# zhudongmei/glusterfs

Measured on AMD Instinct MI355X. Metric: EC encode/decode user-data GB/s (4+2, 8+4) at 1/2/4/8 MI355X; % HBM roofline, higher is better.
Workload: dtype u8

## Files before the change

glusterfs_amd/csrc/ec_jit.hip:

```cpp
#include <hip/hip_runtime.h>

#include <dlfcn.h>
#include <fcntl.h>
#include <spawn.h>
#include <sys/wait.h>
#include <unistd.h>
#include <pthread.h>
#include <errno.h>
#include <stdarg.h>
#include <stdint.h>
#include <stdio.h>
#include <stdlib.h>
#include <string.h>

#include <atomic>
#include <chrono>
#include <condition_variable>
#include <deque>
#include <mutex>
#include <new>
#include <string>
#include <thread>
#include <vector>

#include "ec_device.h"
#include "ec_jit.h"

extern char **environ;

namespace {

using u32 = uint32_t;
constexpr int kMaxDev = 16;
constexpr size_t kEntries = 32;
constexpr uint64_t kMaxCreated = 256;


u32 gf_mul(u32 a, u32 b)
{
    u32 r = 0;
    while (b) {
        if (b & 1)
            r ^= a;
        a <<= 1;
        if (a & 0x100)
            a ^= 0x11D;
        b >>= 1;
    }
    return r;
}

u32 plane_mask(u32 c, int b)
{
    u32 m = 0;
    for (int j = 0; j < 8; ++j)
        m |= ((gf_mul(c, 1u << j) >> b) & 1u) << j;
    return m;
}

struct Gen {
    std::string s;
    u32 ops = 0;

    void line(const char *fmt, ...) __attribute__((format(printf, 2, 3)))
    {
        char buf[256];
        va_list ap, aq;
        va_start(ap, fmt);
        va_copy(aq, ap);
        const int n = vsnprintf(buf, sizeof buf, fmt, ap);
        va_end(ap);
        if (n >= (int)sizeof buf) {
            std::string big((size_t)n + 1, '\0');
            vsnprintf(&big[0], big.size(), fmt, aq);
            big.resize((size_t)n);
            s += big;
        } else if (n > 0) {
            s += buf;
        }
        va_end(aq);
        s += '\n';
    }
};

void emit_program(Gen &g, int w, u32 k, u32 T, const uint8_t *coef, u32 r0, u32 r1)
{
    const u32 ps = T * 64u;
    const u32 no = (r1 - r0) * 8;
    g.line("__device__ __forceinline__ void prog%d(u32 col, u32 *acc)", w);
    g.line("{");
    g.line("    asm volatile(\"\" : \"+v\"(col));");
    std::string decl = "    u32 x0, x1, x2, x3, x4, x5, x6, x7, n0, n1, n2, n3, n4, n5, n6, n7";
    for (u32 o = 0; o < no; ++o)
        decl += ", a" + std::to_string(o);
    g.line("%s;", decl.c_str());
    for (int b = 0; b < 8; ++b)
        g.line("    n%d = LDW(col + %uu);", b, (u32)b * ps);
    std::vector<bool> started(no, false);
    for (u32 p = 0; p < k; ++p) {
        g.line("    x0 = n0; x1 = n1; x2 = n2; x3 = n3; x4 = n4; x5 = n5; x6 = n6; x7 = n7;");
        if (p + 1 < k)
            for (int b = 0; b < 8; ++b)
                g.line("    n%d = LDW(col + %uu);", b, ((p + 1) * 8 + (u32)b) * ps);
        g.line("    __builtin_amdgcn_sched_barrier(0);");
        g.line("    {");
        std::vector<u32> masks(no);
        for (u32 o = 0; o < no; ++o)
            masks[o] = plane_mask(coef[(size_t)(r0 + o / 8) * k + p], (int)(o % 8));
        for (int h = 0; h < 2; ++h) {
            bool need[16] = {};
            for (u32 o = 0; o < no; ++o)
                need[(masks[o] >> (4 * h)) & 15] = true;
            bool have[16] = {};
            for (int j = 0; j < 4; ++j) {
                g.line("        const u32 t%d_%d = x%d;", h, 1 << j, 4 * h + j);
                have[1 << j] = true;
            }
            for (int pc = 2; pc <= 4; ++pc)
                for (int m = 1; m < 16; ++m) {
                    if (__builtin_popcount(m) != pc || !(need[m] || (pc == 2 && m == 3 && need[15])))
                        continue;
                    if (have[m])
                        continue;
                    int bits[4], nb = 0;
                    for (int j = 0; j < 4; ++j)
                        if (m >> j & 1)
                            bits[nb++] = 1 << j;
                    if (pc == 2)
                        g.line("        const u32 t%d_%d = t%d_%d ^ t%d_%d;", h, m, h, bits[0], h, bits[1]);
                    else if (pc == 3)
                        g.line("        const u32 t%d_%d = xr3(t%d_%d, t%d_%d, t%d_%d);", h, m, h, bits[0],
                               h, bits[1], h, bits[2]);
                    else
                        g.line("        const u32 t%d_15 = xr3(t%d_3, t%d_4, t%d_8);", h, h, h, h);
                    have[m] = true;
                    ++g.ops;
                }
        }
        for (u32 o = 0; o < no; ++o) {
            const u32 m0 = masks[o] & 15, m1 = masks[o] >> 4;
            char t0[16] = "", t1[16] = "";
            if (m0)
                snprintf(t0, sizeof t0, "t0_%u", m0);
            if (m1)
                snprintf(t1, sizeof t1, "t1_%u", m1);
            if (!m0 && !m1)
                continue;
            if (!started[o]) {
                if (m0 && m1) {
                    g.line("        a%u = %s ^ %s;", o, t0, t1);
                    ++g.ops;
                } else {
                    g.line("        a%u = %s;", o, m0 ? t0 : t1);
                }
                started[o] = true;
            } else if (m0 && m1) {
                g.line("        a%u = xr3(a%u, %s, %s);", o, o, t0, t1);
                ++g.ops;
            } else {
                g.line("        a%u ^= %s;", o, m0 ? t0 : t1);
                ++g.ops;
            }
        }
        g.line("    }");
        g.line("    __builtin_amdgcn_sched_barrier(0);");
    }
    for (u32 o = 0; o < no; ++o)
        g.line("    acc[%u] = %s;", o, started[o] ? ("a" + std::to_string(o)).c_str() : "0u");
    g.line("}");
}

const char *kPrologue = R"(
typedef unsigned int u32;
typedef unsigned long long u64;
typedef u32 v4u __attribute__((ext_vector_type(4)));
#define LDW(off) (*(const __attribute__((address_space(3))) u32 *)(off))
__device__ __forceinline__ u32 xr3(u32 a, u32 b, u32 c)
{
    return __builtin_amdgcn_bitop3_b32(a, b, c, 0x96);
}
struct JitArgs {
    const unsigned char *in[16];
    unsigned char *out[16];
    u64 in_stride, out_stride, nstripes;
    u64 contig;    /* out[r] = out[0] + r * 512 and out_stride = ROWS * 512 */
};
)";

const char *kBody = R"(
template <int LA>
__device__ __forceinline__ void body(const JitArgs &a)
{
    extern __shared__ __attribute__((aligned(16))) unsigned char lds[];
    constexpr u32 NW = T / 2u, PER = T / 2u, NT = NW * 64u;
    const u32 tid = threadIdx.x, lane = tid & 63u;
    const u32 wave = __builtin_amdgcn_readfirstlane(tid >> 6);
    const u64 t0 = (u64)blockIdx.x * T;
    /* the shipped tile kernels' staging (ec_kernels_impl.h stage_tile): input
     * p, plane b, stripe s at ((p * 8 + b) * T + s) * 64 */
    for (u32 ins = wave; ins < K * PER; ins += NW) {
        const u32 p = ins / PER, el = (ins % PER) * 64u + lane, seg = el >> 2;
        const u64 st = t0 + seg % T;
        if (st < a.nstripes) {
            const unsigned char *gp = a.in[p] + st * a.in_stride + (seg / T) * 64u + (el & 3u) * 16u;
            __builtin_amdgcn_global_load_lds((const __attribute__((address_space(1))) void *)gp,
                                             (__attribute__((address_space(3))) void *)(lds + ins * 1024u),
                                             16, 0, LA);
        }
    }
    /* every wave's LDS-DMA has landed before any wave reads the tile: the
     * hiprtc build of __syncthreads() waits only for lgkmcnt (the product
     * build adds vmcnt(0) itself), so the wait is explicit */
    __builtin_amdgcn_s_waitcnt(0x0070);          /* vmcnt(0) lgkmcnt(0) */
    __syncthreads();
    /* wave w: rows half (w & 1), stripes 4 * (w >> 1) .. + 3 */
    const u32 half = wave & 1u, s = (wave >> 1) * 4u + (lane >> 4), cc = lane & 15u;
    const u32 col = (u32)(unsigned long long)(lds + s * 64u + cc * 4u);
    u32 acc[NA];
    if (half == 0)
        prog0(col, acc);
    else
        prog1(col, acc);
    __syncthreads();
    /* stripe s, row r at (s * ROWS + r) * 512: a full decode's tile is then
     * its output as it lies in memory (ec_method_decode's stripe-major out) */
    unsigned char *ob = lds + s * (ROWS * 512u) + cc * 4u;
    const u32 rb = half == 0 ? 0u : R0;
    const u32 nr = half == 0 ? R0 : ROWS - R0;
#pragma unroll
    for (u32 o = 0; o < NA; ++o)
        if (o < nr * 8u)
            *(u32 *)(ob + (rb + o / 8u) * 512u + (o % 8u) * 64u) = acc[o];
    __syncthreads();
    const u64 left = a.nstripes - t0;
    const u32 ns = (u32)(left < T ? left : T);
    if (a.contig) {
        /* one run of ns * ROWS * 512 bytes */
        unsigned char *o = a.out[0] + t0 * a.out_stride;
        for (u32 i = tid * 16u; i < ns * ROWS * 512u; i += NT * 16u)
            __builtin_nontemporal_store(*(const v4u *)(lds + i), (v4u *)(o + i));
    } else {
        /* row by row: 512-byte runs, one per stripe (fragment-major outputs) */
        for (u32 r = 0; r < ROWS; ++r) {
            const u32 ss = tid >> 5, q = tid & 31u;
            if (ss < ns)
                __builtin_nontemporal_store(*(const v4u *)(lds + (ss * ROWS + r) * 512u + q * 16u),
                                            (v4u *)(a.out[r] + (t0 + ss) * a.out_stride + q * 16u));
        }
    }
}
extern "C" __global__ __launch_bounds__(T / 2 * 64) void ec_jit_combine(JitArgs a) { body<0>(a); }
extern "C" __global__ __launch_bounds__(T / 2 * 64) void ec_jit_combine_nt(JitArgs a) { body<2>(a); }
)";


struct Compiler {
    std::string path, why;
    bool ok = false;

    Compiler()
    {
        if (const char *e = getenv("EC_MI355X_JITC")) {
            path = e;
        } else {
            Dl_info di;
            if (dladdr((const void *)&ecd_jit_stats, &di) && di.dli_fname) {
                path = di.dli_fname;
                const size_t sl = path.rfind('/');
                path = (sl == std::string::npos ? std::string(".") : path.substr(0, sl)) +
                       "/ec_jitc";
            }
        }
        ok = !path.empty() && access(path.c_str(), X_OK) == 0;
        if (!ok)
            why = "compiler " + (path.empty() ? std::string("ec_jitc") : path) + " not found";
    }
};

Compiler &compiler()
{
    static Compiler *c = new Compiler;
    return *c;
}

bool read_file(const std::string &p, std::vector<char> &out)
{
    FILE *f = fopen(p.c_str(), "rb");
    if (!f)
        return false;
    char buf[1 << 16];
    size_t n;
    out.clear();
    while ((n = fread(buf, 1, sizeof buf, f)) > 0)
        out.insert(out.end(), buf, buf + n);
    fclose(f);
    return true;
}

int run_compiler(const std::string &src, std::vector<char> &code, std::string &log)
{
    Compiler &c = compiler();
    if (!c.ok) {
        log = c.why;
        return -ENOSYS;
    }
    const char *tmp = getenv("TMPDIR");
    std::string base = std::string(tmp && *tmp ? tmp : "/tmp") + "/ec_jit_XXXXXX";
    std::vector<char> name(base.begin(), base.end());
    name.push_back('\0');
    const int fd = mkstemp(name.data());
    if (fd < 0) {
        log = "mkstemp failed";
        return -EIO;
    }
    const std::string sp(name.data()), cp = sp + ".co", lp = sp + ".log";
    const bool wrote = write(fd, src.data(), src.size()) == (ssize_t)src.size();
    close(fd);
    int rc = -EIO;
    if (wrote) {
        posix_spawn_file_actions_t fa;
        posix_spawn_file_actions_init(&fa);
        posix_spawn_file_actions_addopen(&fa, 1, "/dev/null", O_WRONLY, 0);
        posix_spawn_file_actions_addopen(&fa, 2, lp.c_str(), O_WRONLY | O_CREAT | O_TRUNC, 0600);
        char *argv[] = {const_cast<char *>(c.path.c_str()), const_cast<char *>(sp.c_str()),
                        const_cast<char *>(cp.c_str()), nullptr};
        pid_t pid = -1;
        if (posix_spawn(&pid, c.path.c_str(), &fa, nullptr, argv, environ) == 0) {
            int st = 0;
            while (waitpid(pid, &st, 0) < 0 && errno == EINTR) {
            }
            if (WIFEXITED(st) && WEXITSTATUS(st) == 0 && read_file(cp, code) && !code.empty())
                rc = 0;
            else
                rc = WIFEXITED(st) && WEXITSTATUS(st) == 2 ? -ENOSYS : -EIO;
        } else {
            log = "posix_spawn of the compiler failed";
        }
        posix_spawn_file_actions_destroy(&fa);
        if (rc) {
            std::vector<char> l;
            if (read_file(lp, l))
                log += std::string(l.begin(), l.end());
        }
    }
    unlink(sp.c_str());
    unlink(cp.c_str());
    unlink(lp.c_str());
    return rc;
}


struct Key {
    u32 k = 0, rows = 0;
    uint8_t coef[ECJ_MAX * ECJ_MAX] = {};
    bool operator==(const Key &o) const
    {
        return k == o.k && rows == o.rows && !memcmp(coef, o.coef, (size_t)k * rows);
    }
};

enum { kQueued = 0, kReady = 1, kFailed = 2 };

struct Entry {
    Key key;
    std::atomic<int> state{kQueued};
    std::vector<char> code;
    hipModule_t mod[kMaxDev] = {};
    hipFunction_t fn[kMaxDev][2] = {};
    int load_failed[kMaxDev] = {};
    uint64_t last_use = 0;
};

struct Jit {
    std::mutex mu;
    std::condition_variable cv;
    std::vector<Entry *> entries;
    std::deque<Entry *> queue;
    bool worker = false;
    uint64_t tick = 0;
    uint64_t created = 0;
    std::atomic<uint64_t> compiled{0}, failed{0}, launches{0}, compile_us{0}, lookups{0};
    std::string last_log;
};

Jit &jit()
{
    static Jit *j = new Jit;
    return *j;
}

long env_long(const char *name, long dflt)
{
    const char *e = getenv(name);
    return e && *e ? strtol(e, nullptr, 10) : dflt;
}

bool jit_on()
{
    static const bool v = env_long("EC_MI355X_JIT", 1) != 0;
    return v;
}

bool jit_sync()
{
    static const bool v = env_long("EC_MI355X_JIT_SYNC", 0) != 0;
    return v;
}

constexpr u32 kJitTile = 4;
u32 jit_tile()
{
    return kJitTile;
}

uint64_t jit_min_stripes()
{
    static const uint64_t v = (uint64_t)env_long("EC_MI355X_JIT_MIN_STRIPES", 1024);
    return v;
}

std::string source_of(const Key &key, u32 *ops)
{
    Gen g;
    const u32 r0 = (key.rows + 1) / 2;
    g.s += kPrologue;
    g.line("#define K %uu", key.k);
    g.line("#define ROWS %uu", key.rows);
    g.line("#define R0 %uu", r0);
    g.line("#define NA %uu", r0 * 8);
    g.line("#define T %uu", jit_tile());

    emit_program(g, 0, key.k, jit_tile(), key.coef, 0, r0);
    emit_program(g, 1, key.k, jit_tile(), key.coef, r0, key.rows);
    g.s += kBody;
    if (ops)
        *ops = g.ops;
    return g.s;
}

void compile_entry(Entry *e)
{
    Jit &j = jit();
    const auto t0 = std::chrono::steady_clock::now();
    u32 ops = 0;
    const std::string src = source_of(e->key, &ops);
    std::string log;
    const int st = run_compiler(src, e->code, log) == 0 ? kReady : kFailed;
    j.compile_us += (uint64_t)std::chrono::duration_cast<std::chrono::microseconds>(
                        std::chrono::steady_clock::now() - t0).count();
    (st == kReady ? j.compiled : j.failed)++;
    if (st != kReady) {
        std::lock_guard<std::mutex> g(j.mu);
        j.last_log = log.substr(0, 2000);
    }
    e->state.store(st, std::memory_order_release);
}

std::thread *g_worker;
bool g_stop;

void worker_main()
{
    Jit &j = jit();
    for (;;) {
        Entry *e;
        {
            std::unique_lock<std::mutex> g(j.mu);
            j.cv.wait(g, [&] { return g_stop || !j.queue.empty(); });
            if (g_stop)
                return;
            e = j.queue.front();
            j.queue.pop_front();
        }
        compile_entry(e);
    }
}

void fork_prepare()
{
    jit().mu.lock();
}

void fork_parent()
{
    jit().mu.unlock();
}

void fork_child()
{
    Jit &j = jit();
    new (&j.mu) std::mutex();
    new (&j.cv) std::condition_variable();
    j.queue.clear();
    j.worker = false;
    g_worker = nullptr;
}

Entry *lookup(const Key &key)
{
    Jit &j = jit();
    Entry *fresh = nullptr;
    {
        std::lock_guard<std::mutex> g(j.mu);
        for (Entry *e : j.entries)
            if (e->key == key) {
                e->last_use = ++j.tick;
                return e;
            }
        if (j.entries.size() >= kEntries) {
            size_t lru = j.entries.size();
            for (size_t i = 0; i < j.entries.size(); ++i)
                if (j.entries[i]->state.load() != kQueued &&
                    (lru == j.entries.size() || j.entries[i]->last_use < j.entries[lru]->last_use))
                    lru = i;
            if (lru == j.entries.size())
                return nullptr;
            j.entries.erase(j.entries.begin() + (long)lru);
        }
        if (j.created >= kMaxCreated)
            return nullptr;
        ++j.created;
        fresh = new Entry;
        fresh->key = key;
        fresh->last_use = ++j.tick;
        j.entries.push_back(fresh);
        if (!jit_sync()) {
            j.queue.push_back(fresh);
            if (!j.worker) {
                static std::once_flag once;
                std::call_once(once, [] { pthread_atfork(fork_prepare, fork_parent, fork_child); });
                g_worker = new std::thread(worker_main);
                j.worker = true;
            }
            j.cv.notify_one();
        }
    }
    if (jit_sync())
        compile_entry(fresh);
    return fresh;
}

hipFunction_t function_of(Entry *e, bool nt)
{
    int dev = 0;
    if (hipGetDevice(&dev) != hipSuccess || dev < 0 || dev >= kMaxDev) {
        (void)hipGetLastError();
        return nullptr;
    }
    Jit &j = jit();
    std::lock_guard<std::mutex> g(j.mu);
    if (e->load_failed[dev])
        return nullptr;
    if (!e->mod[dev]) {
        hipModule_t m = nullptr;
        hipFunction_t f0 = nullptr, f1 = nullptr;
        if (hipModuleLoadData(&m, e->code.data()) != hipSuccess ||
            hipModuleGetFunction(&f0, m, "ec_jit_combine") != hipSuccess ||
            hipModuleGetFunction(&f1, m, "ec_jit_combine_nt") != hipSuccess) {
            (void)hipGetLastError();
            e->load_failed[dev] = 1;
            return nullptr;
        }
        e->mod[dev] = m;
        e->fn[dev][0] = f0;
        e->fn[dev][1] = f1;
    }
    return e->fn[dev][nt ? 1 : 0];
}

struct JitArgs {
    const uint8_t *in[16];
    uint8_t *out[16];
    uint64_t in_stride, out_stride, nstripes;
    uint64_t contig;
};

}

extern "C" int ecj_lds_pad_kb = 0;

extern "C" int ecj_eligible(const ecd_combine_desc_t *d)
{
    if (!jit_on() || d->npatterns != 1 || d->group_pattern || d->k < 12 || d->k > ECJ_MAX ||
        d->rows < 12 || d->rows > ECJ_MAX || d->nstripes < jit_min_stripes() ||
        d->nstripes / 4 + 1 > 0x7fffffffull)
        return 0;
    if (d->out_stride % 16)
        return 0;
    for (uint32_t r = 0; r < d->rows; ++r)
        if (!d->out_base[r] || ((uintptr_t)d->out_base[r] & 15))
            return 0;
    return 1;
}

extern "C" int ecj_launch(hipStream_t s, const ecd_combine_desc_t *d, int nt)
{
    if (!ecj_eligible(d) || !compiler().ok)
        return -EAGAIN;
    const uint8_t *pat = d->pat_ext ? d->pat_ext : d->pat;
    Key key;
    key.k = d->k;
    key.rows = d->rows;
    memcpy(key.coef, pat + d->k, (size_t)d->rows * d->k);
    jit().lookups++;
    Entry *e = lookup(key);
    if (!e || e->state.load(std::memory_order_acquire) != kReady)
        return -EAGAIN;
    hipFunction_t f = function_of(e, nt != 0);
    if (!f)
        return -EAGAIN;
    JitArgs a;
    memset(&a, 0, sizeof a);
    for (uint32_t p = 0; p < d->k; ++p) {
        a.in[p] = static_cast<const uint8_t *>(d->in_base[pat[p]]);
        if (!a.in[p])
            return -EAGAIN;
    }
    for (uint32_t r = 0; r < d->rows; ++r)
        a.out[r] = static_cast<uint8_t *>(d->out_base[r]);
    a.in_stride = d->in_stride;
    a.out_stride = d->out_stride;
    a.nstripes = d->nstripes;
    a.contig = d->out_stride == (uint64_t)d->rows * 512;
    for (uint32_t r = 1; r < d->rows && a.contig; ++r)
        a.contig = a.out[r] == a.out[0] + (size_t)r * 512;
    const u32 T = jit_tile();
    const size_t lds = (size_t)(d->k > d->rows ? d->k : d->rows) * T * 512 +
                       (size_t)ecj_lds_pad_kb * 1024;
    if (lds > (64u << 10))
        return -EAGAIN;
    void *params[] = {&a};
    const hipError_t rc = hipModuleLaunchKernel(f, (u32)((d->nstripes + T - 1) / T), 1, 1, T / 2 * 64,
                                                1, 1, (u32)lds, s, params, nullptr);
    if (rc != hipSuccess) {
        (void)hipGetLastError();
        return -EAGAIN;
    }
    jit().launches++;
    return 0;
}

extern "C" void ecd_jit_stats(ecd_jit_stats_t *st)
{
    Jit &j = jit();
    st->compiled = j.compiled.load();
    st->failed = j.failed.load();
    st->launches = j.launches.load();
    st->compile_us = j.compile_us.load();
    st->lookups = j.lookups.load();
    std::lock_guard<std::mutex> g(j.mu);
    st->entries = j.entries.size();
}

extern "C" int ecd_jit_prepare(uint32_t k, uint32_t rows, const uint8_t *coef)
{
    if (k < 1 || k > ECJ_MAX || rows < 2 || rows > ECJ_MAX || !coef)
        return -EINVAL;
    if (!jit_on())
        return -EPERM;
    if (!compiler().ok)
        return -ENOSYS;
    Key key;
    key.k = k;
    key.rows = rows;
    memcpy(key.coef, coef, (size_t)k * rows);
    return lookup(key) ? 0 : -ENOSPC;
}

extern "C" int ecd_jit_source(uint32_t k, uint32_t rows, const uint8_t *coef, char *buf, size_t len)
{
    if (k < 1 || k > ECJ_MAX || rows < 2 || rows > ECJ_MAX || !coef)
        return -EINVAL;
    Key key;
    key.k = k;
    key.rows = rows;
    memcpy(key.coef, coef, (size_t)k * rows);
    const std::string src = source_of(key, nullptr);
    if (buf && len) {
        const size_t n = src.size() < len - 1 ? src.size() : len - 1;
        memcpy(buf, src.data(), n);
        buf[n] = '\0';
    }
    return (int)(src.size() + 1);
}

extern "C" int ecd_jit_compile_check(uint32_t k, uint32_t rows, const uint8_t *coef, uint32_t *ops,
                                 char *log, size_t log_len)
{
    if (k < 1 || k > ECJ_MAX || rows < 2 || rows > ECJ_MAX || !coef)
        return -EINVAL;
    if (!compiler().ok) {
        if (log && log_len)
            snprintf(log, log_len, "%s", compiler().why.c_str());
        return -ENOSYS;
    }
    Entry e;
    e.key.k = k;
    e.key.rows = rows;
    memcpy(e.key.coef, coef, (size_t)k * rows);
    const std::string src = source_of(e.key, ops);
    compile_entry(&e);
    if (const char *d = getenv("EC_MI355X_JIT_DUMP")) {
        if (FILE *f = fopen((std::string(d) + ".hip").c_str(), "w")) {
            fwrite(src.data(), 1, src.size(), f);
            fclose(f);
        }
        if (!e.code.empty())
            if (FILE *f = fopen((std::string(d) + ".co").c_str(), "wb")) {
                fwrite(e.code.data(), 1, e.code.size(), f);
                fclose(f);
            }
    }
    if (e.state.load() != kReady && log && log_len) {
        std::lock_guard<std::mutex> g(jit().mu);
        snprintf(log, log_len, "%s", jit().last_log.c_str());
    }
    return e.state.load() == kReady ? (int)e.code.size() : -EIO;
}
```

Measured before the change: 3323.

## Extend JIT GF(2^8) combine kernel to narrow k<=8 codes with row groups and searched XOR programs

Result: slower. 3193 (-3.9%).

```diff
diff --git a/glusterfs_amd/csrc/ec_gf8_prog_tab.h b/glusterfs_amd/csrc/ec_gf8_prog_tab.h
--- /dev/null
+++ b/glusterfs_amd/csrc/ec_gf8_prog_tab.h
@@ -0,0 +1,281 @@
+#ifndef EC_MI355X_GF8_PROG_TAB_H
+#define EC_MI355X_GF8_PROG_TAB_H
+
+static const unsigned short ecgf_prog_off[256] = {
+    0, 0, 17, 37, 66, 90, 121, 152, 189, 215, 249, 281, 320, 351, 391, 430,
+    469, 499, 528, 564, 602, 635, 672, 712, 752, 786, 823, 860, 898, 936, 976, 1016,
+    1057, 1091, 1123, 1153, 1181, 1218, 1253, 1293, 1325, 1362, 1398, 1434, 1469, 1507, 1548, 1587,
+    1626, 1660, 1697, 1733, 1771, 1809, 1848, 1884, 1923, 1960, 1996, 2034, 2071, 2114, 2152, 2192,
+    2231, 2267, 2302, 2339, 2368, 2405, 2436, 2463, 2487, 2524, 2562, 2598, 2636, 2676, 2712, 2744,
+    2778, 2815, 2849, 2886, 2920, 2957, 2997, 3028, 3066, 3105, 3143, 3182, 3221, 3257, 3298, 3335,
+    3374, 3409, 3447, 3486, 3527, 3563, 3600, 3641, 3680, 3719, 3759, 3799, 3837, 3870, 3906, 3945,
+    3983, 4019, 4056, 4091, 4128, 4165, 4201, 4238, 4276, 4317, 4358, 4394, 4431, 4471, 4511, 4550,
+    4588, 4626, 4667, 4700, 4739, 4776, 4816, 4845, 4883, 4920, 4960, 4993, 5031, 5060, 5096, 5116,
+    5145, 5183, 5222, 5258, 5298, 5335, 5375, 5413, 5450, 5490, 5529, 5565, 5601, 5634, 5667, 5699,
+    5732, 5772, 5811, 5848, 5887, 5927, 5964, 5997, 6032, 6069, 6103, 6146, 6185, 6214, 6241, 6276,
+    6309, 6350, 6388, 6426, 6463, 6500, 6541, 6578, 6613, 6649, 6687, 6727, 6765, 6803, 6842, 6880,
+    6922, 6956, 6989, 7026, 7064, 7105, 7142, 7184, 7222, 7257, 7288, 7327, 7365, 7405, 7444, 7483,
+    7525, 7564, 7603, 7644, 7682, 7722, 7757, 7794, 7832, 7861, 7896, 7931, 7970, 8009, 8044, 8083,
+    8121, 8158, 8195, 8231, 8271, 8306, 8343, 8383, 8421, 8460, 8500, 8533, 8569, 8606, 8644, 8680,
+    8718, 8756, 8796, 8837, 8873, 8909, 8943, 8983, 9016, 9056, 9097, 9137, 9170, 9208, 9246, 9285,
+};
+
+static const signed char ecgf_prog_tab[] = {
+     0, 1, 0, 1, 1, 1, 2, 1, 3, 1, 4, 1, 5, 1, 6, 1, 7,
+     0, 1, 7, 1, 0, 2, 7, 1, 2, 7, 2, 2, 7, 3, 1, 4, 1, 5, 1, 6,
+     1, 2, 7, -1, 2, 7, 0, 2, 1, 0, 2, 8, 1, 2, 8, 3, 3, 7, 4, 3, 2, 5, 4, 2, 6, 5, 2, 7, 6,
+     1, 6, 7, -1, 1, 6, 1, 7, 2, 6, 0, 2, 8, 1, 2, 8, 2, 2, 7, 3, 1, 4, 1, 5,
+     0, 2, 6, 0, 2, 7, 1, 3, 6, 2, 0, 4, 7, 6, 3, 1, 4, 7, 6, 4, 2, 3, 7, 5, 3, 2, 6, 4, 2, 7, 5,
+     1, 2, 6, -1, 2, 7, 6, 2, 7, 0, 4, 7, 6, 1, 0, 2, 8, 1, 2, 8, 3, 3, 7, 4, 3, 2, 5, 4, 2, 6, 5,
+     4, 6, 7, -1, 0, 1, 8, 2, 3, 6, 4, 5, 7, 2, 8, 0, 2, 9, 6, 2, 9, 2, 2, 10, 1, 2, 10, 4, 2, 11, 3, 2, 11, 8, 2, 8, 5,
+     0, 1, 5, 1, 6, 2, 7, 5, 3, 6, 5, 0, 4, 7, 6, 5, 1, 3, 7, 6, 2, 2, 7, 3, 1, 4,
+     2, 2, 5, 7, 6, 7, -1, 2, 5, 0, 2, 6, 1, 1, 8, 4, 6, 5, 3, 0, 4, 9, 5, 4, 1, 2, 8, 6, 2, 9, 3, 2, 7, 4,
+     1, 2, 6, 7, 2, 7, 5, 2, 6, 0, 2, 5, 1, 3, 8, 5, 0, 4, 6, 5, 3, 1, 2, 8, 4, 3, 7, 5, 3, 2, 6, 4,
+     3, 5, 6, 7, 4, 8, -1, 0, 6, -1, 2, 10, 8, 2, 10, 1, 3, 5, 2, 1, 4, 8, 3, 2, 0, 4, 9, 7, 3, 1, 2, 9, 2, 2, 8, 3, 2, 9, 5,
+     1, 0, 5, 7, 2, 6, 5, 2, 7, 6, 2, 8, 6, 2, 8, 1, 3, 5, 2, 1, 3, 6, 3, 2, 3, 7, 4, 3, 2, 5, 4,
+     4, 5, 7, -1, 0, 6, 8, 1, 2, 5, 1, 3, 6, 2, 9, 7, 3, 7, 6, 1, 2, 9, 2, 2, 11, 9, 2, 10, 4, 2, 11, 10, 4, 11, 7, 4, 1, 2, 8, 4,
+     4, 0, 1, 5, 5, 6, -1, 1, 7, 9, 2, 3, 6, 2, 10, 1, 2, 10, 8, 2, 8, 6, 2, 8, 2, 2, 11, 10, 2, 11, 4, 4, 7, 5, 4, 3, 2, 9, 4,
+     4, 5, 6, 7, 0, 1, 5, 3, 4, 8, 2, 9, -1, 2, 8, 0, 2, 9, 8, 2, 11, 6, 2, 11, 3, 4, 10, 6, 2, 1, 3, 10, 7, 2, 1, 10, 2, 10, 3,
+     2, 4, 5, 6, 6, 7, -1, 1, 4, 1, 5, 2, 6, 4, 2, 9, 8, 2, 8, 0, 3, 9, 5, 1, 2, 9, 2, 2, 7, 3,
+     0, 2, 4, 0, 2, 5, 1, 3, 6, 4, 2, 4, 7, 5, 4, 3, 3, 6, 5, 0, 3, 7, 6, 1, 2, 7, 2, 1, 3,
+     4, 5, 6, 7, 1, 4, 8, 1, 3, 9, 4, 5, -1, 2, 7, 4, 2, 5, 0, 2, 9, 5, 2, 11, 2, 2, 10, 0, 1, 9, 2, 8, 2, 2, 11, 10,
+     4, 0, 5, -1, 4, 7, -1, 1, 6, 9, 2, 4, 5, 2, 9, 0, 2, 8, 1, 2, 10, 2, 2, 11, 3, 4, 8, 7, 6, 3, 1, 10, 2, 11, 9, 2, 6, 3,
+     2, 1, 5, 6, 2, 4, 7, 2, 6, 4, 2, 7, 5, 2, 4, 0, 2, 8, 4, 3, 9, 5, 0, 2, 8, 3, 2, 9, 6, 3, 7, 5, 3,
+     4, 0, 4, -1, 0, 2, 7, 1, 5, -1, 3, 6, 10, 2, 8, 6, 2, 10, 7, 2, 8, 2, 2, 11, 4, 2, 9, 5, 2, 11, 5, 2, 9, 8, 2, 5, 3,
+     4, 4, 5, -1, 5, 6, 7, 0, 4, 7, 2, 4, 9, 2, 9, 8, 2, 10, 8, 2, 10, 1, 2, 11, 1, 4, 8, 3, 2, 0, 4, 8, 6, 3, 1, 1, 11, 2, 9, 3,
+     4, 2, 4, 7, 1, 8, -1, 3, 5, 6, 0, 2, 6, 2, 11, 8, 4, 7, 5, 1, 0, 2, 9, 0, 2, 10, 9, 2, 11, 10, 4, 6, 4, 3, 1, 2, 8, 5, 1, 10,
+     2, 4, 6, 7, 3, 6, -1, 2, 5, 4, 2, 6, 5, 2, 8, 5, 2, 8, 0, 4, 7, 4, 1, 0, 3, 5, 2, 1, 2, 9, 2, 2, 9, 8,
+     4, 0, 4, -1, 6, 7, 8, 0, 5, 9, 1, 4, 7, 2, 8, 5, 2, 11, 10, 2, 10, 2, 2, 9, 3, 2, 11, 8, 2, 2, 1, 2, 3, 2, 2, 4, 3,
+     4, 0, 1, 4, 0, 5, 6, 2, 4, 5, 3, 4, 6, 3, 10, 7, 2, 1, 9, 2, 9, 8, 2, 10, 9, 2, 8, 3, 2, 10, 1, 2, 11, 10, 2, 11, 7,
+     3, 2, 4, -1, 1, 5, 6, 3, 6, 8, 4, 7, 5, 4, 0, 2, 9, 0, 2, 9, 8, 2, 10, 0, 3, 3, 1, 0, 2, 8, 1, 3, 5, 3, 2, 2, 10, 2,
+     4, 4, 5, 7, 4, 6, -1, 0, 1, 9, 2, 3, 4, 2, 9, 5, 2, 9, 8, 2, 8, 0, 2, 10, 6, 2, 10, 2, 3, 11, 8, 1, 2, 11, 6, 2, 8, 3,
+     4, 0, 4, 5, 3, 4, -1, 1, 3, 8, 2, 7, 8, 2, 8, 6, 4, 7, 6, 5, 1, 1, 11, 2, 10, 5, 4, 6, 2, 1, 0, 2, 11, 10, 2, 9, 2, 2, 9, 5,
+     4, 2, 4, -1, 5, 6, 7, 3, 8, 9, 0, 1, 5, 2, 9, 4, 2, 9, 0, 2, 11, 4, 4, 8, 7, 1, 0, 2, 11, 10, 3, 10, 6, 1, 2, 10, 7, 2, 10, 2,
+     5, 0, 1, 7, 2, 3, 8, 3, 4, 5, 9, 10, -1, 2, 6, 11, 2, 12, 1, 2, 12, 4, 2, 11, 7, 2, 9, 4, 2, 9, 6, 3, 9, 4, 0, 2, 10, 2, 2, 10, 6,
+     1, 3, 5, -1, 2, 7, 3, 1, 4, 2, 8, 7, 4, 7, 6, 4, 3, 2, 8, 4, 4, 6, 5, 4, 0, 4, 7, 6, 5, 1, 3, 7, 6, 2,
+     1, 4, 6, -1, 3, 7, 3, 0, 2, 4, 1, 4, 7, 5, 3, 2, 2, 8, 7, 2, 5, 3, 2, 8, 0, 3, 7, 5, 1, 2, 6, 2,
+     0, 1, 3, 2, 4, 0, 3, 5, 3, 1, 4, 6, 4, 3, 2, 3, 7, 5, 4, 3, 6, 5, 0, 3, 7, 6, 1, 2, 7, 2,
+     0, 2, 3, 0, 3, 4, 1, 0, 4, 5, 3, 2, 1, 3, 6, 4, 2, 2, 7, 5, 2, 6, 0, 2, 7, 1, 1, 2,
+     4, 5, 6, 7, 1, 4, -1, 3, 4, 8, 1, 9, 10, 2, 11, 5, 2, 7, 4, 2, 11, 0, 2, 9, 3, 2, 10, 2, 2, 10, 0, 2, 9, 8, 2, 8, 2,
+     4, 3, 6, 7, 1, 4, 7, 2, 5, -1, 0, 8, -1, 1, 11, 1, 9, 2, 11, 10, 2, 4, 1, 2, 10, 8, 2, 11, 4, 2, 9, 5, 2, 10, 6,
+     4, 0, 3, 5, 4, 7, -1, 1, 6, -1, 2, 4, 5, 2, 6, 3, 2, 9, 0, 2, 10, 8, 4, 9, 3, 2, 1, 2, 11, 6, 3, 8, 7, 6, 2, 10, 9, 2, 11, 9,
+     2, 0, 3, 6, 1, 4, 7, 1, 8, 2, 9, 0, 4, 8, 5, 2, 1, 2, 9, 2, 3, 6, 5, 2, 2, 8, 7, 1, 9, 2, 5, 2,
+     3, 3, 7, -1, 4, 5, 8, 1, 5, 6, 2, 9, 4, 2, 6, 4, 1, 3, 2, 9, 0, 2, 10, 9, 4, 9, 3, 2, 0, 2, 10, 3, 4, 7, 6, 4, 2,
+     2, 0, 4, 7, 4, 6, -1, 4, 7, 5, 3, 0, 2, 9, 1, 2, 3, 2, 2, 8, 5, 4, 7, 6, 3, 1, 2, 8, 2, 3, 5, 3, 1, 2, 9, 2,
+     3, 0, 2, 5, 1, 3, -1, 4, 6, -1, 2, 5, 3, 2, 10, 0, 2, 9, 7, 3, 8, 4, 3, 2, 10, 1, 2, 8, 7, 2, 9, 6, 3, 7, 4, 2,
+     2, 0, 3, -1, 2, 3, 7, 2, 8, 5, 4, 6, 4, 1, 0, 2, 9, 1, 4, 5, 4, 2, 0, 2, 6, 1, 2, 9, 8, 2, 3, 1, 2, 4, 2,
+     4, 3, 5, 6, 2, 3, 4, 0, 5, -1, 1, 4, 8, 2, 8, 7, 3, 7, 6, 4, 2, 10, 8, 2, 11, 0, 2, 9, 1, 2, 10, 9, 1, 11, 3, 9, 8, 7,
+     4, 0, 2, 3, 0, 1, -1, 1, 3, 5, 4, 5, 6, 4, 10, 9, 7, 6, 4, 7, 6, 4, 1, 2, 8, 6, 2, 11, 9, 2, 9, 8, 2, 8, 4, 2, 10, 4, 2, 11, 2,
+     4, 1, 3, 6, 2, 4, 7, 0, 2, 6, 1, 5, 8, 1, 11, 2, 10, 9, 3, 8, 7, 0, 4, 11, 9, 1, 0, 2, 9, 1, 2, 11, 10, 2, 8, 4, 2, 9, 5,
+     4, 1, 7, -1, 0, 6, 8, 2, 3, -1, 2, 4, 5, 4, 6, 5, 3, 0, 2, 9, 4, 2, 10, 9, 2, 11, 9, 2, 8, 2, 2, 10, 0, 3, 4, 3, 1, 1, 11,
+     2, 3, 6, -1, 4, 7, 8, 2, 9, 6, 2, 5, 4, 2, 9, 5, 2, 8, 5, 2, 8, 0, 4, 7, 4, 1, 0, 3, 5, 2, 1, 2, 8, 2,
+     3, 0, 4, 7, 3, 6, 7, 1, 5, -1, 2, 8, 3, 2, 10, 4, 4, 9, 5, 4, 2, 2, 6, 5, 2, 9, 8, 2, 10, 8, 3, 10, 6, 2, 2, 9, 2,
+     3, 0, 7, -1, 4, 5, -1, 3, 6, 9, 2, 4, 3, 2, 9, 0, 2, 10, 1, 4, 10, 7, 4, 2, 2, 8, 6, 2, 8, 1, 2, 2, 1, 2, 3, 2,
+     4, 1, 2, 6, 1, 5, 7, 0, 4, 7, 3, 7, -1, 2, 11, 10, 2, 10, 9, 4, 8, 5, 4, 3, 2, 9, 8, 2, 10, 6, 2, 9, 0, 1, 8, 2, 11, 2,
+     5, 4, 5, 7, 1, 3, 4, 3, 5, 6, 0, 3, 8, 2, 4, 5, 2, 10, 8, 1, 8, 1, 11, 2, 9, 8, 2, 12, 11, 2, 9, 0, 2, 12, 1, 2, 10, 2,
+     5, 3, 4, 7, 0, 8, -1, 1, 5, 7, 2, 5, -1, 4, 6, 11, 2, 9, 6, 2, 10, 4, 2, 11, 9, 1, 10, 2, 9, 2, 2, 10, 9, 2, 12, 1, 2, 12, 8,
+     4, 2, 3, 5, 3, 4, -1, 1, 5, 9, 0, 4, 5, 2, 9, 6, 2, 11, 7, 2, 10, 0, 2, 8, 1, 2, 2, 0, 2, 11, 10, 2, 10, 8, 1, 8,
+     3, 0, 3, 4, 1, 5, 8, 2, 8, -1, 2, 8, 6, 3, 9, 7, 3, 2, 9, 2, 2, 10, 9, 2, 10, 3, 2, 9, 4, 4, 6, 4, 2, 1, 4, 7, 5, 3, 2,
+     3, 3, 5, 7, 4, 6, -1, 1, 8, -1, 2, 8, 4, 2, 9, 5, 2, 9, 3, 2, 3, 0, 2, 10, 0, 4, 9, 2, 1, 0, 2, 10, 2, 3, 9, 3, 2,
+     4, 1, 4, 5, 2, 3, 6, 0, 3, 8, 4, 7, 9, 3, 10, 7, 1, 2, 8, 6, 2, 9, 4, 1, 0, 2, 10, 7, 2, 10, 9, 2, 11, 8, 1, 11,
+     2, 3, 4, -1, 2, 3, 7, 2, 8, 5, 4, 6, 5, 4, 0, 4, 8, 7, 6, 1, 2, 9, 0, 3, 5, 1, 0, 4, 6, 2, 1, 0, 2, 9, 1, 2, 8, 2,
+     4, 0, 4, 5, 1, 6, -1, 2, 4, 9, 3, 7, 10, 2, 8, 3, 2, 9, 8, 1, 11, 3, 7, 2, 0, 2, 8, 1, 2, 10, 8, 2, 11, 4, 2, 11, 9,
+     6, 3, 4, -1, 6, 7, 8, 2, 5, 6, 0, 1, 9, 1, 3, 10, 3, 9, -1, 2, 9, 5, 2, 13, 5, 2, 8, 0, 2, 11, 4, 2, 12, 0, 2, 11, 2, 2, 13, 12, 2, 10, 8,
+     4, 4, 5, 6, 0, 2, 3, 7, 8, 9, 1, 10, -1, 2, 10, 2, 2, 11, 9, 2, 9, 4, 4, 7, 6, 1, 0, 2, 11, 7, 1, 11, 2, 11, 0, 2, 10, 0,
+     5, 0, 1, 3, 2, 6, 8, 4, 7, -1, 0, 6, 10, 3, 4, 5, 2, 12, 6, 2, 11, 5, 2, 10, 8, 1, 9, 3, 12, 10, 9, 2, 9, 7, 2, 11, 9, 2, 12, 2,
+     4, 0, 1, 6, 4, 7, 8, 2, 3, 9, 5, 10, -1, 4, 11, 7, 2, 1, 2, 9, 5, 2, 10, 6, 2, 8, 2, 2, 11, 3, 2, 11, 4, 2, 10, 0, 2, 11, 8,
+     2, 2, 6, 7, 3, 4, -1, 1, 8, 2, 7, 3, 2, 8, 4, 4, 6, 5, 3, 2, 2, 9, 2, 2, 9, 5, 4, 6, 5, 4, 0, 4, 8, 5, 2, 1,
+     3, 5, 6, -1, 0, 4, -1, 0, 6, 7, 2, 10, 2, 3, 7, 3, 1, 2, 10, 9, 2, 8, 2, 2, 3, 2, 2, 4, 3, 2, 9, 5, 2, 8, 1,
+     4, 0, 6, -1, 3, 6, 7, 1, 2, 4, 1, 7, -1, 2, 6, 2, 2, 9, 8, 2, 10, 6, 2, 9, 5, 2, 11, 10, 2, 5, 3, 2, 8, 4, 2, 11, 5,
+     0, 3, 6, 2, 0, 4, 7, 3, 1, 0, 3, 6, 4, 1, 3, 7, 6, 5, 2, 7, 2, 1, 3, 2, 4, 0, 2, 5, 1,
+     3, 1, 7, -1, 0, 4, 7, 0, 5, -1, 2, 7, 2, 1, 3, 2, 9, 2, 4, 8, 5, 3, 2, 4, 9, 6, 3, 0, 2, 10, 9, 2, 10, 6, 2, 8, 6,
+     1, 0, 7, -1, 2, 8, 2, 2, 3, 1, 2, 8, 4, 4, 7, 5, 2, 1, 3, 7, 6, 3, 2, 7, 4, 2, 5, 0, 2, 6, 1,
+     0, 1, 2, 2, 3, 0, 4, 4, 2, 1, 0, 3, 5, 3, 1, 2, 6, 4, 2, 7, 5, 2, 6, 0, 2, 7, 1,
+     1, 0, 1, -1, 2, 2, 0, 2, 8, 3, 2, 8, 4, 2, 5, 1, 1, 6, 1, 7, 1, 0, 1, 1,
+     4, 4, 5, 6, 2, 7, 8, 0, 2, 3, 1, 9, -1, 2, 9, 4, 3, 7, 6, 3, 2, 8, 2, 1, 10, 2, 11, 3, 2, 9, 3, 2, 10, 9, 2, 11, 2,
+     3, 3, 6, 7, 4, 5, 6, 0, 8, -1, 4, 10, 5, 3, 2, 2, 8, 1, 1, 9, 2, 2, 0, 4, 8, 5, 2, 1, 3, 8, 4, 2, 2, 10, 9, 2, 9, 1,
+     4, 2, 5, 6, 0, 3, 7, 1, 4, 7, 7, 8, -1, 1, 8, 2, 9, 6, 2, 10, 8, 1, 9, 2, 11, 10, 2, 11, 3, 3, 9, 6, 4, 2, 10, 5,
+     4, 0, 3, 7, 0, 2, 6, 1, 5, 6, 4, 10, -1, 2, 9, 5, 3, 8, 6, 1, 2, 11, 7, 2, 7, 0, 2, 10, 2, 2, 9, 8, 2, 8, 4, 2, 11, 6,
+     3, 0, 3, 6, 2, 4, 5, 5, 7, -1, 2, 10, 2, 2, 8, 0, 2, 9, 0, 4, 8, 7, 2, 1, 4, 9, 3, 2, 1, 2, 9, 6, 2, 10, 8, 4, 7, 6, 4, 1,
+     2, 1, 6, -1, 0, 2, 7, 2, 9, 5, 2, 8, 3, 3, 5, 4, 0, 2, 9, 8, 3, 5, 3, 1, 3, 6, 4, 2, 4, 7, 5, 3, 0, 2, 8, 4,
+     2, 0, 3, 6, 1, 4, 7, 2, 5, 2, 1, 8, 4, 9, 5, 2, 0, 2, 8, 1, 2, 9, 5, 3, 6, 5, 2, 2, 8, 7, 1, 9,
+     3, 0, 1, 6, 0, 5, -1, 1, 7, 9, 2, 9, 2, 2, 8, 3, 2, 10, 4, 1, 8, 2, 10, 0, 2, 6, 2, 3, 7, 3, 0, 2, 4, 1,
+     4, 3, 5, 6, 5, 7, -1, 4, 8, 9, 0, 2, 8, 3, 10, 3, 2, 2, 9, 3, 2, 7, 2, 2, 10, 2, 1, 11, 2, 10, 1, 2, 11, 10, 2, 8, 1,
+     4, 2, 4, 6, 3, 5, 7, 0, 7, 8, 1, 6, 9, 1, 10, 2, 9, 1, 1, 7, 2, 10, 0, 2, 10, 9, 2, 11, 4, 2, 10, 5, 1, 11,
+     3, 0, 5, 7, 4, 6, -1, 2, 4, 8, 2, 9, 2, 2, 8, 3, 2, 2, 1, 2, 9, 3, 2, 10, 9, 4, 7, 6, 3, 1, 2, 10, 5, 3, 5, 3, 1,
+     4, 0, 2, 4, 1, 3, 5, 6, 7, 8, 7, 9, -1, 2, 8, 6, 2, 11, 0, 1, 1, 2, 6, 4, 2, 10, 5, 2, 11, 6, 1, 10, 1, 11,
+     4, 0, 5, 7, 1, 3, 4, 4, 6, -1, 2, 6, 7, 2, 11, 10, 2, 5, 3, 2, 11, 0, 2, 9, 2, 2, 8, 3, 2, 10, 1, 2, 8, 2, 2, 10, 9,
+     4, 0, 7, -1, 2, 4, -1, 1, 3, 6, 3, 4, 5, 2, 9, 8, 3, 5, 3, 1, 2, 8, 6, 2, 9, 1, 2, 11, 8, 2, 11, 10, 4, 8, 6, 5, 2, 2, 10, 7,
+     0, 2, 4, 2, 3, 5, 3, 0, 4, 6, 2, 1, 0, 4, 7, 4, 3, 1, 2, 5, 0, 2, 6, 1, 3, 7, 2, 0, 2, 3, 1,
+     3, 0, 4, -1, 1, 6, -1, 1, 7, -1, 2, 8, 2, 4, 5, 3, 1, 0, 2, 9, 0, 2, 10, 4, 2, 8, 5, 2, 9, 5, 4, 7, 6, 2, 0, 2, 10, 3,
+     4, 2, 3, 4, 3, 5, 6, 0, 5, 8, 1, 4, -1, 3, 9, 8, 7, 2, 9, 7, 2, 5, 2, 2, 10, 7, 4, 11, 8, 7, 0, 2, 8, 1, 1, 10, 2, 11, 9,
+     5, 0, 2, 4, 1, 3, 7, 5, 6, 9, 7, 8, 10, 6, 11, -1, 2, 11, 9, 1, 10, 1, 5, 2, 12, 9, 2, 9, 8, 2, 12, 0, 2, 11, 1, 2, 10, 4,
+     5, 0, 3, 5, 2, 4, 5, 1, 2, 3, 0, 10, -1, 7, 8, -1, 2, 9, 6, 2, 12, 6, 2, 12, 11, 2, 8, 4, 2, 11, 3, 1, 10, 2, 9, 8, 2, 10, 9,
+     4, 0, 2, 4, 1, 3, 5, 5, 8, -1, 7, 9, -1, 2, 10, 6, 3, 11, 6, 0, 2, 11, 3, 2, 10, 2, 2, 8, 1, 2, 9, 2, 3, 8, 6, 3, 2, 11, 4,
+     3, 0, 2, 5, 1, 3, 6, 2, 4, 7, 2, 10, 5, 3, 9, 5, 1, 2, 8, 6, 3, 9, 8, 4, 2, 9, 0, 2, 10, 1, 2, 8, 3, 2, 9, 4,
+     4, 1, 4, 5, 3, 5, 6, 0, 9, -1, 7, 8, -1, 4, 11, 2, 1, 0, 2, 9, 1, 2, 10, 3, 4, 8, 6, 2, 0, 2, 10, 8, 2, 11, 2, 2, 10, 2, 2, 11, 9,
+     3, 0, 5, 6, 1, 7, 8, 3, 4, -1, 3, 5, 4, 2, 2, 8, 3, 2, 9, 2, 2, 10, 9, 2, 9, 5, 3, 7, 2, 1, 3, 3, 2, 0, 2, 10, 1,
+     5, 1, 5, 7, 0, 6, 8, 0, 2, 3, 3, 4, 5, 3, 9, -1, 2, 11, 10, 2, 12, 7, 1, 9, 2, 9, 4, 2, 12, 11, 2, 8, 2, 2, 10, 6, 2, 11, 8,
+     2, 3, 6, -1, 2, 4, 5, 2, 8, 2, 3, 7, 4, 3, 2, 9, 8, 2, 9, 7, 2, 5, 2, 2, 8, 0, 4, 7, 4, 1, 0, 3, 5, 2, 1,
+     4, 0, 3, 6, 3, 4, 5, 1, 5, 7, 2, 9, -1, 2, 8, 2, 2, 10, 9, 2, 9, 6, 2, 11, 7, 2, 11, 3, 2, 8, 5, 3, 10, 9, 8, 2, 10, 2,
+     4, 2, 3, 7, 0, 3, 4, 1, 2, 5, 8, 10, -1, 2, 8, 6, 2, 9, 7, 4, 11, 6, 4, 2, 2, 5, 4, 2, 8, 5, 2, 9, 6, 2, 11, 9, 2, 10, 6,
+     5, 4, 5, 7, 3, 8, -1, 1, 6, 8, 0, 1, 9, 7, 10, 11, 2, 12, 2, 2, 11, 5, 2, 10, 3, 2, 9, 7, 2, 9, 2, 2, 12, 8, 2, 10, 0, 3, 10, 4, 2,
+     3, 0, 7, -1, 5, 6, -1, 2, 4, 9, 2, 3, 2, 2, 4, 3, 4, 10, 6, 3, 0, 2, 10, 1, 2, 9, 7, 2, 8, 6, 2, 8, 1, 2, 2, 1,
+     3, 0, 6, 7, 0, 4, 5, 0, 2, 3, 1, 10, 3, 4, 3, 1, 2, 9, 3, 4, 10, 9, 6, 1, 2, 9, 8, 2, 8, 5, 2, 8, 1, 3, 7, 2, 1,
+     5, 1, 5, 7, 4, 8, -1, 0, 3, 9, 1, 6, -1, 3, 5, 11, 3, 7, 3, 2, 2, 10, 8, 2, 10, 2, 2, 9, 6, 2, 12, 1, 2, 12, 10, 2, 8, 0, 2, 11, 2,
+     5, 1, 6, 7, 3, 4, 5, 0, 3, 7, 1, 4, 10, 6, 9, -1, 2, 10, 2, 2, 11, 7, 2, 11, 5, 2, 9, 8, 1, 12, 2, 12, 10, 2, 12, 11, 2, 8, 2,
+     4, 4, 6, 7, 1, 2, 4, 0, 2, 3, 0, 8, -1, 4, 10, 6, 5, 0, 2, 8, 3, 2, 11, 10, 2, 11, 2, 2, 9, 8, 2, 10, 7, 2, 10, 9, 2, 9, 5,
+     5, 1, 4, -1, 3, 6, 7, 0, 2, 9, 2, 7, 8, 5, 10, -1, 2, 12, 7, 2, 9, 8, 2, 9, 4, 2, 10, 4, 2, 11, 6, 2, 12, 6, 2, 11, 10, 2, 11, 5,
+     4, 4, 6, -1, 2, 3, 6, 1, 2, 8, 0, 7, 8, 3, 9, 7, 5, 2, 11, 3, 2, 10, 3, 2, 8, 0, 2, 9, 1, 2, 11, 9, 4, 10, 9, 5, 0, 2, 10, 5,
+     4, 1, 4, 6, 0, 3, 8, 2, 5, 7, 0, 3, 10, 2, 11, 6, 2, 9, 7, 2, 9, 0, 2, 9, 1, 3, 9, 2, 0, 2, 11, 4, 2, 9, 5, 2, 10, 8,
+     3, 1, 2, 4, 2, 3, -1, 0, 4, 9, 2, 9, 5, 3, 6, 4, 3, 2, 10, 7, 2, 8, 0, 1, 1, 2, 2, 0, 2, 10, 8, 1, 8,
+     3, 0, 1, 3, 0, 2, 5, 1, 4, 7, 2, 9, 3, 4, 8, 6, 4, 0, 2, 10, 8, 3, 8, 4, 2, 2, 4, 1, 1, 9, 2, 8, 6, 2, 10, 2,
+     3, 0, 1, 3, 1, 4, 6, 2, 4, -1, 4, 7, 5, 3, 2, 2, 9, 8, 2, 10, 8, 4, 7, 4, 1, 0, 3, 8, 7, 0, 2, 10, 0, 2, 8, 5, 2, 9, 2,
+     5, 1, 3, 4, 0, 8, -1, 0, 2, 5, 3, 7, 10, 5, 6, 9, 1, 11, 2, 12, 5, 1, 9, 2, 9, 7, 2, 8, 7, 2, 10, 4, 2, 12, 4, 2, 12, 11,
+     4, 2, 4, 6, 3, 5, 7, 0, 1, -1, 2, 9, -1, 2, 8, 3, 2, 9, 4, 2, 11, 7, 1, 2, 2, 8, 0, 2, 10, 9, 2, 10, 8, 2, 11, 1,
+     3, 0, 2, 4, 1, 3, 5, 6, 8, -1, 2, 10, 3, 3, 9, 7, 4, 2, 9, 1, 2, 3, 2, 2, 10, 4, 4, 7, 3, 1, 0, 2, 8, 1, 2, 9, 2,
+     4, 2, 3, 7, 1, 5, 8, 0, 2, 9, 4, 6, 8, 1, 11, 3, 10, 4, 1, 1, 9, 1, 7, 2, 11, 0, 2, 10, 4, 2, 11, 10, 2, 9, 6,
+     4, 0, 3, 7, 0, 1, 5, 2, 6, 8, 1, 4, 8, 2, 10, 4, 2, 11, 5, 2, 9, 8, 2, 8, 0, 1, 10, 1, 11, 3, 9, 4, 2, 3, 10, 9, 7,
+     3, 0, 2, 6, 1, 2, 7, 3, 4, -1, 2, 10, 2, 2, 10, 5, 3, 8, 5, 3, 2, 9, 6, 3, 7, 4, 0, 3, 5, 1, 0, 2, 8, 1, 2, 9, 3,
+     1, 1, 2, -1, 4, 4, 3, 2, 0, 4, 5, 4, 3, 1, 4, 6, 5, 3, 0, 4, 8, 7, 6, 3, 2, 7, 0, 2, 1, 0, 2, 8, 0, 2, 8, 3,
+     4, 0, 1, 5, 2, 3, 7, 0, 3, 4, 6, 8, -1, 2, 9, 4, 2, 10, 5, 2, 11, 9, 2, 6, 1, 1, 10, 2, 8, 4, 2, 11, 2, 3, 9, 6, 1,
+     4, 0, 4, -1, 1, 3, 6, 1, 2, 5, 2, 3, 8, 2, 11, 7, 2, 11, 10, 4, 9, 7, 5, 0, 1, 9, 2, 3, 0, 2, 8, 1, 2, 10, 0, 2, 9, 2,
+     5, 2, 3, 7, 4, 5, 8, 6, 9, -1, 0, 1, 3, 2, 5, 6, 2, 10, 7, 2, 10, 2, 1, 8, 2, 12, 0, 2, 11, 9, 2, 12, 11, 4, 10, 5, 1, 0, 2, 9, 1,
+     5, 0, 2, 3, 1, 8, -1, 5, 6, 8, 3, 7, 9, 4, 11, -1, 2, 10, 4, 2, 12, 10, 2, 7, 3, 1, 10, 2, 11, 5, 2, 9, 6, 2, 12, 3, 4, 9, 5, 4, 0,
+     4, 1, 2, 3, 4, 5, 8, 6, 7, 9, 0, 8, 10, 2, 10, 1, 2, 11, 3, 1, 8, 2, 11, 4, 2, 9, 0, 3, 9, 6, 0, 2, 10, 0, 1, 10,
+     4, 0, 3, 5, 1, 2, 8, 4, 6, 9, 7, 10, -1, 2, 11, 1, 2, 11, 2, 2, 3, 1, 3, 8, 7, 6, 1, 9, 2, 10, 5, 2, 11, 6, 2, 10, 0,
+     4, 1, 2, 7, 0, 6, 8, 3, 4, 5, 5, 8, -1, 2, 10, 2, 2, 10, 6, 3, 9, 3, 1, 2, 11, 0, 4, 11, 9, 4, 1, 2, 9, 5, 2, 9, 3, 2, 11, 10,
+     5, 1, 2, 3, 0, 7, 8, 0, 1, 5, 0, 3, 6, 4, 10, -1, 2, 12, 8, 2, 12, 11, 2, 11, 7, 2, 9, 5, 2, 10, 6, 3, 11, 9, 0, 1, 9, 2, 8, 4,
+     4, 0, 5, -1, 3, 6, 8, 1, 2, 9, 4, 7, 10, 4, 11, 6, 1, 0, 2, 9, 4, 2, 10, 5, 2, 8, 1, 2, 11, 2, 2, 11, 3, 2, 11, 4, 2, 11, 8,
+     4, 0, 3, 5, 1, 6, 8, 2, 7, 8, 0, 4, 9, 2, 10, 4, 2, 11, 0, 2, 9, 5, 2, 8, 1, 2, 9, 7, 2, 11, 10, 2, 10, 1, 3, 11, 5, 2,
+     4, 3, 4, -1, 1, 2, 5, 2, 6, 7, 1, 3, 6, 2, 10, 9, 1, 10, 2, 11, 5, 2, 9, 4, 2, 11, 10, 2, 8, 2, 2, 8, 5, 4, 6, 5, 4, 0,
+     4, 1, 2, -1, 3, 4, 5, 6, 7, -1, 0, 5, 10, 2, 11, 1, 2, 10, 8, 4, 8, 6, 5, 3, 2, 9, 8, 4, 8, 7, 4, 3, 2, 9, 2, 2, 9, 6, 2, 11, 4,
+     0, 3, 6, 5, 1, 4, 7, 6, 2, 0, 4, 7, 6, 5, 3, 4, 7, 5, 4, 1, 2, 2, 1, 2, 3, 2, 2, 4, 3, 3, 5, 4, 0,
+     4, 2, 7, -1, 3, 5, 8, 0, 1, 6, 1, 2, 4, 2, 10, 5, 2, 10, 8, 2, 9, 6, 2, 11, 9, 1, 11, 2, 9, 7, 3, 6, 4, 3, 4, 7, 5, 4, 0,
+     4, 5, 7, -1, 2, 4, 8, 0, 1, 3, 0, 6, -1, 2, 8, 1, 2, 6, 2, 2, 10, 5, 2, 9, 6, 2, 11, 10, 2, 9, 5, 2, 5, 3, 2, 11, 4,
+     4, 2, 4, 7, 3, 5, 6, 0, 2, 6, 1, 10, -1, 4, 7, 5, 1, 0, 2, 11, 0, 2, 11, 9, 2, 9, 8, 4, 6, 4, 3, 1, 2, 8, 5, 1, 9, 2, 10, 8,
+     0, 2, 5, 1, 3, 6, 2, 0, 4, 7, 5, 3, 0, 3, 6, 5, 4, 3, 7, 6, 1, 2, 7, 2, 1, 3, 2, 4, 0,
+     4, 0, 5, -1, 2, 7, 8, 0, 1, 6, 0, 4, 7, 2, 8, 1, 2, 10, 2, 2, 9, 3, 4, 6, 5, 4, 3, 2, 11, 10, 2, 9, 0, 2, 6, 3, 1, 11,
+     4, 0, 6, -1, 1, 6, 7, 3, 5, 6, 4, 5, 7, 1, 9, 2, 7, 2, 2, 9, 3, 4, 8, 4, 2, 1, 2, 10, 2, 2, 11, 10, 1, 11, 2, 8, 5,
+     4, 5, 6, 7, 2, 7, -1, 0, 1, 6, 3, 4, 8, 2, 10, 7, 2, 9, 1, 4, 10, 9, 3, 0, 4, 10, 4, 3, 2, 2, 11, 9, 1, 11, 2, 11, 3, 2, 8, 0,
+     1, 0, 7, -1, 2, 6, 1, 2, 8, 2, 2, 6, 3, 4, 8, 6, 4, 1, 4, 7, 6, 5, 2, 3, 7, 6, 3, 2, 7, 4, 2, 5, 0,
+     3, 2, 6, -1, 0, 1, 2, 4, 7, 8, 2, 9, 8, 2, 9, 7, 2, 8, 3, 3, 10, 9, 3, 2, 10, 5, 4, 7, 6, 5, 3, 2, 10, 2, 3, 7, 5, 0,
+     0, 2, 7, 1, 1, 2, 4, 7, 3, 1, 0, 4, 7, 4, 2, 0, 3, 7, 5, 3, 2, 6, 4, 2, 7, 5, 2, 6, 0,
+     3, 0, 7, -1, 2, 3, 8, 5, 6, -1, 2, 8, 1, 2, 2, 1, 2, 9, 1, 2, 9, 4, 4, 7, 5, 4, 3, 2, 10, 4, 2, 10, 7, 2, 8, 6,
+     0, 1, 1, 2, 2, 0, 2, 3, 0, 2, 4, 0, 1, 5, 1, 6, 1, 7, 1, 0,
+     1, 0, 2, -1, 2, 1, 0, 2, 8, 1, 2, 8, 3, 3, 4, 3, 0, 2, 5, 4, 2, 6, 5, 2, 7, 6, 2, 7, 0,
+     4, 3, 4, 5, 6, 7, 8, 1, 2, -1, 2, 3, 9, 2, 11, 10, 2, 11, 4, 2, 8, 1, 2, 10, 7, 3, 10, 9, 0, 2, 10, 9, 2, 9, 2, 2, 9, 0,
+     4, 1, 2, 7, 5, 8, -1, 3, 4, 9, 0, 6, 10, 3, 11, 3, 2, 2, 9, 6, 2, 10, 7, 2, 8, 3, 2, 11, 4, 3, 11, 5, 0, 2, 10, 1, 2, 11, 8,
+     4, 2, 5, 6, 3, 4, 7, 1, 4, 8, 5, 9, -1, 2, 10, 2, 3, 8, 7, 0, 1, 11, 1, 1, 2, 10, 0, 2, 10, 9, 2, 11, 8, 2, 11, 0,
+     5, 1, 6, -1, 0, 5, 8, 2, 3, 7, 2, 7, -1, 3, 4, 5, 2, 9, 4, 2, 11, 9, 2, 12, 11, 2, 3, 1, 2, 9, 2, 2, 10, 8, 2, 10, 4, 2, 12, 0,
+     4, 1, 4, 5, 2, 6, -1, 0, 3, 8, 3, 7, 9, 2, 8, 7, 2, 9, 5, 2, 10, 6, 1, 9, 1, 10, 2, 9, 8, 2, 11, 5, 4, 11, 4, 2, 0,
+     4, 0, 1, 5, 1, 2, 6, 1, 3, 9, 4, 8, -1, 2, 11, 7, 2, 9, 5, 2, 11, 10, 1, 10, 2, 8, 3, 2, 9, 4, 4, 7, 5, 3, 2, 4, 10, 4, 2, 0,
+     3, 0, 4, 7, 1, 5, -1, 2, 5, 6, 2, 9, 4, 2, 10, 0, 4, 10, 8, 3, 2, 2, 7, 6, 2, 9, 8, 2, 10, 1, 4, 7, 6, 3, 2, 2, 8, 3,
+     3, 0, 1, 5, 2, 6, -1, 3, 7, 9, 2, 8, 4, 2, 9, 8, 4, 10, 5, 4, 0, 2, 10, 2, 2, 8, 7, 2, 9, 1, 2, 10, 6, 3, 4, 3, 0,
+     4, 1, 3, 4, 2, 5, 6, 0, 2, 3, 7, 9, -1, 4, 7, 6, 4, 1, 2, 11, 6, 2, 8, 7, 3, 11, 1, 0, 2, 10, 4, 2, 8, 5, 2, 9, 4, 2, 11, 10,
+     4, 1, 4, -1, 1, 2, 5, 0, 3, 6, 3, 7, 8, 2, 11, 10, 2, 9, 7, 2, 11, 2, 3, 10, 9, 7, 3, 3, 2, 0, 2, 8, 3, 2, 9, 8, 2, 10, 5,
+     2, 0, 2, 7, 4, 6, -1, 2, 9, 1, 2, 8, 5, 2, 4, 3, 4, 6, 5, 1, 0, 2, 8, 4, 3, 5, 3, 1, 2, 9, 2, 4, 7, 5, 3, 0,
+     2, 0, 5, -1, 2, 7, 8, 4, 6, 4, 1, 0, 2, 9, 1, 3, 4, 3, 2, 4, 8, 6, 3, 1, 2, 9, 5, 2, 3, 1, 2, 4, 2, 2, 8, 3,
+     3, 0, 3, 6, 1, 4, 7, 2, 5, -1, 1, 9, 1, 10, 2, 9, 8, 2, 10, 0, 3, 9, 8, 1, 2, 9, 5, 2, 10, 6, 2, 8, 7,
+     2, 0, 3, 6, 1, 4, 7, 2, 9, 0, 3, 5, 2, 1, 3, 9, 8, 2, 4, 5, 3, 2, 0, 2, 8, 7, 1, 9, 2, 5, 2, 1, 8,
+     2, 0, 4, 6, 0, 5, -1, 2, 4, 1, 2, 9, 2, 2, 8, 3, 2, 9, 7, 1, 8, 3, 7, 5, 1, 2, 6, 2, 3, 7, 3, 0,
+     1, 0, 4, -1, 2, 8, 1, 4, 5, 2, 1, 0, 4, 8, 6, 3, 2, 4, 7, 5, 3, 0, 2, 6, 0, 2, 7, 1, 1, 2, 2, 3, 0,
+     5, 2, 5, 6, 4, 6, 7, 1, 9, -1, 0, 8, -1, 1, 3, 8, 2, 12, 2, 2, 9, 2, 2, 10, 4, 2, 12, 7, 2, 10, 8, 2, 11, 3, 2, 10, 3, 2, 11, 9,
+     5, 1, 2, 7, 6, 8, -1, 0, 2, 3, 3, 4, 7, 5, 7, 10, 2, 12, 9, 2, 9, 4, 1, 9, 2, 9, 5, 2, 8, 5, 2, 10, 6, 2, 11, 1, 2, 12, 11,
+     4, 1, 3, 5, 4, 6, 7, 0, 2, 9, 4, 8, -1, 2, 11, 9, 1, 10, 1, 6, 2, 8, 6, 2, 11, 2, 4, 10, 8, 7, 1, 2, 9, 8, 2, 10, 5,
+     4, 0, 2, 6, 1, 3, 5, 4, 8, -1, 7, 8, 9, 2, 11, 2, 3, 10, 7, 1, 2, 8, 0, 3, 6, 5, 1, 2, 9, 2, 2, 10, 3, 2, 11, 10, 2, 10, 5,
+     3, 0, 7, -1, 2, 4, -1, 3, 5, -1, 2, 10, 1, 2, 9, 6, 2, 8, 1, 2, 10, 2, 4, 6, 5, 4, 1, 4, 8, 6, 5, 2, 4, 7, 6, 3, 1, 2, 9, 8,
+     3, 0, 2, 7, 1, 6, -1, 2, 4, -1, 4, 5, 3, 1, 0, 2, 10, 9, 2, 8, 1, 2, 5, 2, 2, 9, 5, 2, 8, 6, 3, 7, 3, 1, 2, 10, 0,
+     4, 3, 5, 7, 0, 2, 4, 1, 6, 8, 6, 7, 9, 2, 8, 1, 2, 9, 6, 1, 0, 1, 8, 2, 10, 4, 2, 11, 5, 1, 10, 1, 11,
+     4, 0, 2, 4, 1, 3, 5, 6, 8, -1, 7, 9, -1, 2, 11, 0, 2, 10, 1, 2, 2, 0, 2, 7, 5, 2, 11, 6, 2, 10, 7, 1, 11, 1, 10,
+     3, 1, 6, -1, 0, 2, 7, 2, 4, -1, 2, 8, 3, 2, 10, 7, 2, 8, 5, 3, 9, 3, 1, 2, 10, 6, 4, 7, 5, 3, 0, 2, 8, 4, 2, 9, 5,
+     3, 1, 2, 7, 0, 1, 6, 0, 2, 5, 2, 9, 3, 2, 8, 4, 2, 10, 9, 2, 8, 0, 2, 6, 2, 3, 7, 3, 0, 2, 4, 1, 1, 10,
+     6, 6, 7, -1, 0, 4, 7, 1, 3, -1, 0, 2, 5, 1, 5, 6, 9, 10, 12, 2, 10, 8, 2, 9, 2, 2, 8, 5, 2, 10, 0, 2, 13, 11, 2, 13, 6, 2, 12, 4, 2, 11, 8,
+     4, 0, 4, 7, 1, 8, -1, 2, 6, 7, 0, 5, 7, 4, 9, 6, 4, 3, 2, 9, 2, 2, 10, 5, 2, 1, 0, 2, 10, 3, 2, 8, 3, 2, 11, 9, 2, 11, 10,
+     0, 2, 3, 1, 2, 4, 2, 3, 5, 1, 0, 4, 6, 3, 2, 0, 2, 7, 4, 2, 5, 0, 2, 6, 1, 3, 7, 2, 0,
+     0, 3, 3, 1, 0, 3, 4, 2, 1, 4, 5, 2, 1, 0, 3, 6, 2, 0, 1, 7, 1, 0, 1, 1, 2, 2, 0,
+     3, 0, 4, -1, 0, 6, 7, 5, 6, -1, 3, 7, 3, 1, 2, 8, 2, 2, 10, 9, 2, 9, 3, 2, 4, 3, 2, 8, 5, 2, 10, 1, 2, 9, 2,
+     1, 0, 6, -1, 4, 7, 3, 1, 0, 4, 4, 2, 1, 0, 4, 7, 5, 2, 0, 2, 8, 7, 1, 3, 2, 4, 0, 2, 5, 1, 2, 8, 2,
+     5, 1, 2, -1, 3, 4, 8, 0, 7, 8, 2, 5, 6, 4, 7, -1, 2, 11, 9, 2, 12, 11, 2, 12, 1, 2, 9, 6, 2, 10, 6, 2, 10, 3, 1, 9, 4, 9, 5, 1, 0,
+     4, 1, 4, 6, 0, 3, 5, 2, 7, 8, 1, 9, 10, 2, 9, 8, 2, 10, 5, 2, 10, 6, 2, 8, 2, 2, 10, 0, 2, 11, 8, 3, 8, 3, 2, 2, 11, 6,
+     5, 1, 3, 4, 0, 2, 6, 6, 7, 8, 4, 5, 9, 5, 8, -1, 2, 10, 5, 2, 11, 7, 1, 4, 1, 10, 2, 12, 11, 2, 10, 9, 2, 12, 2, 2, 11, 3,
+     4, 1, 4, 6, 0, 2, 8, 3, 5, 9, 7, 10, -1, 2, 11, 2, 2, 11, 3, 2, 4, 2, 2, 8, 7, 2, 9, 3, 2, 11, 6, 2, 10, 0, 2, 11, 1,
+     3, 1, 2, -1, 2, 3, 4, 2, 4, 6, 3, 9, 8, 5, 2, 10, 5, 4, 10, 8, 7, 0, 2, 9, 7, 2, 1, 0, 2, 8, 0, 2, 8, 3, 2, 9, 0,
+     4, 2, 4, -1, 0, 1, 2, 0, 3, 7, 6, 7, 9, 4, 9, 8, 5, 3, 4, 8, 6, 5, 1, 2, 11, 4, 2, 8, 7, 2, 9, 8, 2, 9, 5, 2, 11, 10, 2, 10, 8,
+     3, 0, 2, 4, 6, 8, -1, 1, 3, 5, 3, 10, 7, 4, 2, 9, 5, 2, 9, 2, 2, 4, 3, 4, 7, 3, 1, 0, 2, 8, 1, 2, 10, 2, 2, 9, 3,
+     4, 0, 1, 4, 1, 2, 6, 3, 7, 8, 2, 5, 8, 2, 10, 5, 2, 11, 6, 2, 9, 8, 1, 4, 1, 10, 1, 11, 3, 9, 5, 3, 2, 10, 9,
+     3, 0, 2, 5, 1, 3, 4, 2, 4, 7, 2, 9, 6, 2, 10, 5, 3, 5, 4, 1, 2, 9, 8, 1, 8, 4, 6, 3, 1, 0, 2, 10, 1, 2, 8, 3,
+     5, 2, 4, 5, 1, 8, -1, 0, 2, 3, 6, 9, 10, 5, 7, 10, 2, 11, 5, 2, 9, 7, 1, 9, 2, 9, 0, 2, 8, 0, 2, 11, 4, 2, 12, 11, 1, 12,
+     5, 2, 5, -1, 4, 7, 8, 0, 3, 8, 1, 9, 10, 6, 11, -1, 2, 12, 0, 2, 9, 0, 2, 9, 2, 2, 11, 5, 2, 10, 7, 2, 12, 7, 2, 9, 1, 2, 10, 6,
+     4, 4, 5, 7, 0, 1, 8, 3, 6, 9, 0, 2, 3, 2, 10, 5, 2, 9, 2, 2, 8, 2, 1, 9, 2, 11, 8, 2, 10, 7, 2, 11, 10, 4, 10, 4, 2, 1,
+     4, 0, 6, 7, 4, 5, -1, 1, 2, 7, 2, 8, 9, 3, 4, 3, 1, 2, 9, 2, 2, 11, 10, 2, 11, 3, 2, 8, 5, 2, 8, 1, 1, 10, 3, 3, 2, 0,
+     4, 0, 1, 4, 1, 6, 7, 2, 5, 8, 5, 9, -1, 2, 8, 3, 2, 10, 0, 2, 10, 6, 2, 10, 9, 2, 11, 8, 2, 11, 0, 2, 9, 2, 4, 7, 3, 2, 0,
+     4, 0, 4, 5, 6, 8, -1, 0, 3, 6, 1, 5, 7, 3, 11, 10, 9, 2, 8, 2, 2, 9, 7, 2, 9, 3, 2, 10, 5, 2, 11, 9, 2, 11, 2, 2, 10, 2,
+     5, 0, 4, 5, 3, 6, -1, 6, 7, 8, 1, 5, 10, 2, 8, -1, 2, 11, 9, 2, 12, 1, 2, 10, 2, 2, 8, 6, 2, 9, 8, 2, 10, 1, 2, 12, 11, 4, 9, 7, 2, 0,
+     2, 1, 4, 7, 3, 6, -1, 3, 5, 2, 1, 2, 9, 2, 4, 8, 5, 3, 2, 3, 9, 4, 1, 1, 8, 2, 5, 2, 2, 9, 0, 2, 8, 0,
+     1, 1, 4, -1, 4, 5, 2, 1, 0, 4, 6, 3, 2, 1, 4, 8, 7, 5, 3, 2, 8, 6, 2, 7, 1, 1, 2, 2, 3, 0, 2, 8, 0,
+     4, 1, 4, 7, 2, 4, 5, 0, 3, 6, 3, 8, -1, 2, 9, 8, 2, 10, 2, 2, 9, 3, 3, 11, 6, 2, 2, 11, 7, 1, 9, 2, 10, 5, 2, 11, 10,
+     3, 0, 1, 6, 2, 8, -1, 3, 5, -1, 4, 9, 7, 6, 5, 2, 9, 3, 2, 10, 4, 4, 9, 7, 4, 0, 2, 3, 1, 2, 4, 2, 2, 10, 0, 2, 8, 4,
+     4, 1, 2, 6, 0, 3, 4, 0, 7, -1, 2, 3, 7, 2, 8, 5, 2, 11, 6, 4, 9, 8, 7, 5, 2, 10, 9, 2, 8, 4, 2, 11, 5, 2, 9, 6, 4, 10, 5, 4, 1,
+     3, 0, 1, 5, 2, 6, -1, 3, 7, 9, 2, 9, 8, 2, 10, 1, 4, 10, 8, 4, 2, 2, 7, 4, 2, 9, 1, 2, 10, 6, 3, 4, 3, 0, 2, 8, 4,
+     6, 3, 4, 6, 2, 6, -1, 0, 5, 8, 5, 7, 9, 0, 3, 5, 1, 7, 8, 2, 11, 1, 2, 12, 11, 2, 10, 2, 2, 9, 8, 2, 13, 2, 2, 11, 8, 1, 10, 2, 13, 12,
+     4, 0, 4, 5, 2, 3, 7, 1, 6, 9, 6, 8, -1, 4, 10, 5, 3, 0, 2, 10, 0, 2, 11, 3, 2, 4, 2, 1, 10, 2, 9, 4, 2, 8, 3, 2, 11, 1,
+     3, 0, 7, -1, 1, 3, 4, 5, 6, -1, 2, 2, 1, 2, 3, 2, 2, 9, 2, 3, 9, 5, 0, 2, 10, 4, 2, 10, 7, 2, 8, 6, 2, 8, 1,
+     1, 1, 2, -1, 2, 8, 0, 2, 8, 3, 3, 4, 3, 1, 4, 5, 4, 1, 0, 2, 6, 5, 2, 7, 6, 2, 7, 0, 2, 1, 0,
+     5, 3, 4, 7, 0, 2, -1, 0, 6, 7, 5, 6, 8, 1, 6, 9, 2, 12, 10, 2, 9, 3, 2, 8, 2, 2, 12, 11, 1, 11, 2, 11, 3, 2, 10, 5, 2, 10, 1,
+     4, 0, 1, 2, 4, 7, -1, 0, 6, -1, 5, 6, 7, 2, 8, 7, 2, 8, 3, 2, 9, 3, 3, 9, 8, 5, 2, 11, 3, 2, 9, 6, 2, 11, 10, 2, 10, 1,
+     4, 0, 4, 6, 2, 3, 8, 2, 5, 7, 3, 5, -1, 3, 6, 2, 1, 2, 11, 10, 2, 9, 1, 2, 10, 9, 2, 10, 4, 2, 11, 6, 2, 8, 7, 4, 10, 2, 1, 0,
+     4, 0, 6, 7, 4, 8, -1, 1, 2, 7, 1, 5, -1, 2, 10, 8, 2, 10, 3, 4, 9, 7, 3, 1, 2, 9, 5, 2, 11, 10, 2, 6, 3, 2, 9, 6, 2, 11, 0,
+     4, 0, 5, 7, 2, 3, 5, 4, 6, 9, 6, 8, -1, 4, 7, 6, 2, 1, 2, 9, 8, 2, 10, 8, 2, 10, 0, 2, 9, 4, 2, 10, 2, 2, 11, 4, 2, 11, 1,
+     5, 2, 3, -1, 0, 7, 8, 2, 4, 6, 3, 6, 9, 4, 5, 7, 2, 11, 1, 2, 9, 1, 2, 10, 9, 2, 12, 11, 2, 8, 5, 2, 10, 8, 2, 12, 0, 4, 6, 5, 1, 0,
+     4, 1, 6, 7, 2, 3, 5, 1, 3, 4, 5, 8, -1, 2, 10, 9, 2, 9, 6, 2, 9, 8, 2, 11, 3, 2, 11, 0, 2, 8, 2, 4, 7, 3, 2, 0, 2, 10, 0,
+     5, 6, 7, -1, 1, 5, 8, 0, 4, 9, 2, 3, 7, 3, 6, 10, 2, 12, 11, 2, 11, 9, 2, 9, 3, 1, 9, 1, 10, 2, 9, 2, 3, 11, 6, 0, 2, 12, 5,
+     4, 3, 5, 6, 0, 8, -1, 1, 2, -1, 4, 7, 10, 2, 11, 5, 2, 9, 2, 2, 8, 2, 2, 10, 8, 2, 9, 1, 2, 11, 6, 4, 9, 7, 6, 2, 4, 9, 5, 4, 1,
+     4, 0, 3, 6, 1, 2, 5, 1, 4, 8, 4, 7, 9, 2, 11, 0, 2, 9, 8, 3, 8, 5, 0, 2, 9, 6, 2, 10, 5, 2, 11, 6, 2, 11, 10, 2, 10, 7,
+     4, 1, 2, 5, 2, 3, 6, 4, 6, -1, 0, 9, 10, 2, 10, 8, 3, 9, 7, 5, 4, 8, 7, 3, 0, 2, 5, 3, 2, 8, 0, 2, 9, 1, 2, 11, 7, 2, 11, 8,
+     4, 0, 1, 5, 3, 7, 8, 0, 6, 9, 2, 4, 8, 2, 11, 6, 2, 10, 2, 1, 9, 1, 5, 1, 11, 3, 10, 7, 2, 2, 11, 10, 2, 9, 4,
+     3, 0, 3, 5, 2, 7, 8, 1, 4, 6, 4, 10, 9, 3, 0, 2, 9, 6, 2, 8, 2, 2, 9, 0, 2, 9, 1, 3, 10, 3, 2, 2, 9, 4, 2, 10, 8,
+     4, 0, 5, -1, 2, 7, 8, 1, 3, 4, 6, 9, 10, 2, 11, 3, 2, 11, 4, 2, 8, 3, 2, 9, 0, 2, 11, 6, 3, 11, 7, 0, 2, 11, 1, 2, 11, 2,
+     1, 0, 1, 3, 3, 4, 2, 1, 3, 5, 3, 2, 4, 8, 6, 2, 0, 2, 8, 7, 1, 0, 1, 1, 2, 2, 0, 1, 8,
+     3, 0, 1, 7, 0, 1, 2, 1, 6, -1, 2, 9, 4, 4, 9, 5, 3, 0, 2, 10, 3, 1, 8, 2, 4, 0, 2, 5, 1, 2, 10, 9, 2, 8, 3,
+     4, 0, 2, 5, 0, 3, 7, 1, 2, 7, 1, 3, 6, 2, 10, 4, 2, 8, 3, 2, 11, 10, 2, 10, 9, 1, 9, 2, 4, 1, 1, 8, 2, 11, 0,
+     4, 0, 1, -1, 3, 6, 7, 0, 2, 5, 2, 4, 8, 2, 11, 7, 3, 10, 3, 1, 1, 9, 2, 8, 2, 4, 7, 4, 3, 0, 2, 11, 10, 2, 10, 6, 2, 9, 8,
+     5, 0, 1, 3, 0, 3, 6, 2, 3, 7, 0, 8, -1, 2, 4, 8, 2, 12, 9, 2, 10, 5, 2, 8, 2, 1, 9, 2, 10, 9, 2, 11, 7, 2, 12, 11, 2, 8, 5,
+     4, 0, 2, 4, 1, 3, -1, 5, 7, 9, 6, 8, -1, 2, 11, 1, 2, 10, 2, 2, 9, 0, 2, 6, 0, 2, 11, 7, 1, 10, 1, 11, 2, 10, 0,
+     5, 0, 2, 3, 6, 7, -1, 1, 2, 9, 5, 7, 8, 3, 4, 7, 2, 10, 4, 1, 11, 2, 11, 5, 2, 9, 8, 2, 8, 6, 2, 12, 1, 2, 12, 11, 2, 11, 10,
+     4, 0, 2, 6, 1, 7, 8, 3, 5, 9, 4, 8, -1, 2, 9, 4, 2, 10, 6, 3, 7, 3, 0, 2, 9, 1, 2, 11, 3, 2, 11, 10, 2, 11, 5, 2, 10, 2,
+     4, 1, 2, -1, 3, 5, 7, 2, 4, 6, 0, 1, -1, 2, 9, 8, 2, 10, 3, 2, 8, 4, 2, 7, 1, 2, 9, 1, 2, 10, 0, 2, 11, 9, 2, 11, 10,
+     4, 1, 3, 7, 0, 5, 8, 4, 8, -1, 2, 6, 10, 2, 9, 2, 2, 11, 7, 2, 4, 1, 1, 8, 2, 10, 5, 2, 11, 9, 2, 9, 6, 3, 11, 3, 0,
+     2, 0, 2, 4, 6, 8, -1, 4, 5, 3, 2, 1, 2, 9, 3, 3, 8, 7, 0, 2, 2, 1, 2, 5, 1, 2, 9, 4, 4, 7, 3, 1, 0, 2, 8, 1,
+     5, 1, 3, -1, 0, 2, 5, 3, 4, 5, 6, 7, 8, 6, 9, 10, 2, 9, 8, 2, 12, 1, 2, 7, 4, 2, 8, 2, 2, 10, 8, 2, 9, 6, 2, 11, 0, 2, 12, 11,
+     4, 1, 2, 6, 0, 4, 8, 1, 7, 9, 3, 5, 8, 2, 11, 7, 3, 10, 3, 0, 1, 9, 1, 6, 1, 11, 2, 10, 3, 2, 11, 10, 2, 9, 5,
+     4, 1, 4, 6, 0, 5, 7, 2, 3, 8, 9, 10, -1, 2, 11, 4, 2, 10, 7, 2, 8, 0, 2, 6, 3, 2, 10, 5, 2, 11, 1, 2, 11, 2, 2, 11, 3,
+     4, 2, 6, 7, 0, 4, -1, 3, 8, -1, 1, 5, 10, 2, 11, 7, 2, 10, 9, 2, 9, 8, 1, 8, 2, 11, 3, 2, 10, 0, 4, 9, 7, 3, 1, 4, 9, 5, 2, 1,
+     4, 0, 6, 7, 2, 3, 8, 1, 4, 9, 3, 5, 10, 4, 9, 7, 5, 1, 1, 10, 2, 8, 4, 2, 9, 0, 2, 11, 0, 2, 9, 5, 2, 10, 2, 2, 11, 6,
+     4, 0, 1, 6, 4, 7, -1, 2, 3, 7, 5, 8, -1, 2, 10, 1, 2, 10, 9, 4, 9, 5, 2, 1, 2, 11, 7, 2, 6, 3, 2, 9, 0, 2, 11, 6, 2, 8, 2,
+     4, 0, 1, 6, 2, 7, 8, 3, 6, -1, 4, 5, 7, 2, 10, 9, 4, 4, 3, 2, 1, 2, 11, 1, 4, 9, 5, 3, 2, 2, 10, 4, 2, 11, 0, 2, 8, 5, 1, 9,
+     1, 1, 2, -1, 2, 8, 3, 4, 4, 3, 2, 0, 3, 5, 4, 2, 4, 8, 6, 5, 0, 2, 7, 6, 2, 7, 0, 2, 1, 0, 2, 8, 0,
+     3, 0, 1, 2, 3, 6, 8, 4, 6, -1, 2, 8, 3, 2, 10, 9, 2, 5, 4, 2, 9, 5, 2, 10, 7, 3, 7, 5, 0, 3, 6, 1, 0, 2, 8, 7,
+     4, 0, 1, 5, 2, 3, 7, 6, 9, -1, 3, 8, 10, 2, 10, 1, 2, 9, 4, 2, 11, 4, 2, 5, 0, 1, 9, 3, 4, 3, 0, 2, 8, 4, 2, 11, 7,
+     5, 2, 3, 7, 0, 3, 5, 1, 6, 8, 4, 10, -1, 2, 9, 11, 2, 10, 0, 2, 11, 6, 1, 12, 1, 9, 2, 8, 4, 2, 9, 4, 2, 12, 7, 2, 10, 9,
+     4, 0, 2, 5, 4, 8, -1, 1, 2, 3, 3, 5, 9, 2, 10, 6, 2, 11, 7, 2, 9, 6, 2, 8, 7, 1, 2, 2, 3, 0, 2, 11, 10, 2, 8, 1,
+     4, 0, 3, -1, 1, 2, 8, 0, 4, 6, 5, 7, 9, 2, 9, 6, 3, 11, 5, 4, 2, 10, 5, 2, 11, 1, 2, 4, 2, 2, 8, 5, 2, 10, 1, 2, 11, 3,
+     5, 1, 2, 6, 1, 4, 5, 0, 3, 8, 2, 7, 9, 4, 7, 10, 2, 11, 3, 3, 10, 9, 0, 1, 8, 1, 9, 2, 12, 2, 2, 11, 0, 2, 10, 5, 1, 12,
+     5, 1, 3, 4, 0, 2, 8, 7, 9, -1, 2, 5, 6, 4, 5, 10, 2, 12, 4, 2, 11, 8, 2, 6, 1, 2, 8, 5, 2, 12, 11, 2, 10, 3, 2, 12, 7, 2, 9, 6,
+     5, 1, 2, -1, 0, 7, 8, 0, 1, 6, 4, 5, 8, 3, 10, -1, 2, 11, 3, 2, 12, 11, 2, 10, 9, 2, 11, 7, 2, 10, 4, 2, 9, 5, 2, 12, 2, 3, 9, 4, 3,
+     4, 0, 1, 2, 3, 4, 8, 0, 5, 9, 0, 6, -1, 2, 10, 0, 2, 11, 10, 2, 7, 6, 2, 10, 7, 2, 11, 1, 2, 8, 7, 2, 8, 3, 1, 9,
+     4, 2, 3, 4, 0, 1, 8, 5, 6, 7, 9, 10, -1, 2, 11, 0, 2, 10, 8, 3, 2, 1, 0, 2, 10, 4, 1, 9, 2, 9, 5, 2, 11, 7, 1, 11,
+     4, 0, 1, 2, 3, 4, 8, 5, 6, 9, 7, 10, -1, 1, 11, 2, 11, 0, 2, 1, 0, 2, 11, 8, 2, 8, 3, 1, 9, 2, 9, 5, 1, 10,
+     4, 0, 2, -1, 1, 4, 8, 3, 5, 9, 6, 10, -1, 2, 11, 0, 3, 11, 7, 1, 2, 8, 7, 4, 11, 3, 1, 0, 2, 9, 7, 2, 10, 4, 2, 11, 5, 2, 10, 7,
+     3, 0, 1, 2, 3, 4, 8, 5, 6, 9, 1, 10, 2, 10, 7, 2, 7, 0, 3, 10, 1, 0, 2, 8, 7, 2, 8, 3, 1, 9, 2, 9, 5,
+     5, 0, 1, 6, 2, 7, 8, 3, 4, 5, 5, 8, -1, 1, 9, 11, 2, 12, 10, 2, 10, 2, 2, 12, 6, 2, 8, 4, 2, 10, 0, 2, 11, 4, 2, 9, 5, 2, 9, 3,
+     4, 0, 1, 4, 0, 5, -1, 2, 3, 8, 6, 10, -1, 2, 10, 7, 2, 10, 9, 4, 7, 6, 5, 1, 2, 11, 2, 2, 9, 3, 2, 8, 6, 4, 9, 7, 2, 1, 2, 11, 4,
+     5, 0, 1, 6, 2, 7, 8, 2, 5, -1, 0, 4, 7, 3, 6, 9, 2, 12, 11, 4, 10, 4, 3, 0, 2, 10, 6, 2, 9, 4, 2, 11, 5, 2, 8, 5, 1, 9, 1, 12,
+     2, 0, 1, 2, 3, 4, 8, 1, 9, 2, 9, 5, 2, 6, 5, 3, 9, 7, 6, 3, 7, 5, 0, 3, 6, 1, 0, 2, 8, 7, 2, 8, 3,
+     4, 0, 7, -1, 2, 5, 8, 3, 4, 9, 1, 6, 10, 3, 11, 5, 0, 2, 10, 0, 2, 9, 1, 2, 8, 4, 2, 11, 1, 2, 11, 2, 2, 11, 3, 2, 11, 4,
+     4, 0, 1, 7, 3, 4, 8, 2, 5, 9, 4, 6, 10, 3, 9, 6, 2, 2, 10, 0, 2, 8, 5, 2, 9, 1, 2, 11, 1, 2, 9, 6, 2, 10, 3, 2, 11, 7,
+     4, 0, 2, 5, 1, 2, 6, 3, 7, 8, 4, 8, -1, 3, 9, 4, 3, 2, 10, 4, 1, 8, 2, 11, 5, 2, 11, 6, 2, 10, 9, 4, 9, 7, 4, 0, 2, 10, 1,
+     5, 0, 1, 3, 2, 4, 8, 7, 9, -1, 2, 5, 6, 4, 5, 10, 2, 9, 6, 2, 12, 4, 2, 5, 0, 2, 9, 1, 2, 11, 0, 2, 12, 11, 2, 10, 3, 2, 12, 7,
+};
+
+#endif
diff --git a/glusterfs_amd/csrc/ec_jit.hip b/glusterfs_amd/csrc/ec_jit.hip
--- a/glusterfs_amd/csrc/ec_jit.hip
+++ b/glusterfs_amd/csrc/ec_jit.hip
@@ -24,6 +24,7 @@
 #include <vector>
 
 #include "ec_device.h"
+#include "ec_gf8_prog_tab.h"
 #include "ec_jit.h"
 
 extern char **environ;
@@ -82,6 +83,147 @@
         s += '\n';
     }
 };
+
+struct Searched {
+    int nt = 0;
+    int t[8][3] = {};
+    std::vector<int> pk[8];
+};
+
+Searched searched_of(u32 c)
+{
+    Searched q;
+    const signed char *r = ecgf_prog_tab + ecgf_prog_off[c];
+    q.nt = *r++;
+    for (int j = 0; j < q.nt; ++j)
+        for (int i = 0; i < 3; ++i)
+            q.t[j][i] = *r++;
+    for (int b = 0; b < 8; ++b) {
+        const int m = *r++;
+        q.pk[b].assign(r, r + m);
+        r += m;
+    }
+    return q;
+}
+
+std::string sig_name(int s)
+{
+    return (s < 8 ? "x" : "u") + std::to_string(s < 8 ? s : s - 8);
+}
+
+void emit_input_tables(Gen &g, u32 k, u32 p, const uint8_t *coef, u32 r0, u32 r1,
+                       std::vector<bool> &started)
+{
+    const u32 no = (r1 - r0) * 8;
+    std::vector<u32> masks(no);
+    for (u32 o = 0; o < no; ++o)
+        masks[o] = plane_mask(coef[(size_t)(r0 + o / 8) * k + p], (int)(o % 8));
+    for (int h = 0; h < 2; ++h) {
+        bool need[16] = {};
+        for (u32 o = 0; o < no; ++o)
+            need[(masks[o] >> (4 * h)) & 15] = true;
+        bool have[16] = {};
+        for (int j = 0; j < 4; ++j) {
+            g.line("        const u32 t%d_%d = x%d;", h, 1 << j, 4 * h + j);
+            have[1 << j] = true;
+        }
+        for (int pc = 2; pc <= 4; ++pc)
+            for (int m = 1; m < 16; ++m) {
+                if (__builtin_popcount(m) != pc || !(need[m] || (pc == 2 && m == 3 && need[15])))
+                    continue;
+                if (have[m])
+                    continue;
+                int bits[4], nb = 0;
+                for (int j = 0; j < 4; ++j)
+                    if (m >> j & 1)
+                        bits[nb++] = 1 << j;
+                if (pc == 2)
+                    g.line("        const u32 t%d_%d = t%d_%d ^ t%d_%d;", h, m, h, bits[0], h, bits[1]);
+                else if (pc == 3)
+                    g.line("        const u32 t%d_%d = xr3(t%d_%d, t%d_%d, t%d_%d);", h, m, h, bits[0],
+                           h, bits[1], h, bits[2]);
+                else
+                    g.line("        const u32 t%d_15 = xr3(t%d_3, t%d_4, t%d_8);", h, h, h, h);
+                have[m] = true;
+                ++g.ops;
+            }
+    }
+    for (u32 o = 0; o < no; ++o) {
+        const u32 m0 = masks[o] & 15, m1 = masks[o] >> 4;
+        char t0[16] = "", t1[16] = "";
+        if (m0)
+            snprintf(t0, sizeof t0, "t0_%u", m0);
+        if (m1)
+            snprintf(t1, sizeof t1, "t1_%u", m1);
+        if (!m0 && !m1)
+            continue;
+        if (!started[o]) {
+            if (m0 && m1) {
+                g.line("        a%u = %s ^ %s;", o, t0, t1);
+                ++g.ops;
+            } else {
+                g.line("        a%u = %s;", o, m0 ? t0 : t1);
+            }
+            started[o] = true;
+        } else if (m0 && m1) {
+            g.line("        a%u = xr3(a%u, %s, %s);", o, o, t0, t1);
+            ++g.ops;
+        } else {
+            g.line("        a%u ^= %s;", o, m0 ? t0 : t1);
+            ++g.ops;
+        }
+    }
+}
+
+void emit_input_searched(Gen &g, u32 k, u32 p, const uint8_t *coef, u32 r0, u32 r1,
+                         std::vector<bool> &started)
+{
+    for (u32 r = r0; r < r1; ++r) {
+        const u32 c = coef[(size_t)r * k + p];
+        if (!c)
+            continue;
+        const Searched q = searched_of(c);
+        g.line("        {");
+        for (int j = 0; j < q.nt; ++j) {
+            if (q.t[j][2] >= 0)
+                g.line("            const u32 u%d = xr3(%s, %s, %s);", j, sig_name(q.t[j][0]).c_str(),
+                       sig_name(q.t[j][1]).c_str(), sig_name(q.t[j][2]).c_str());
+            else
+                g.line("            const u32 u%d = %s ^ %s;", j, sig_name(q.t[j][0]).c_str(),
+                       sig_name(q.t[j][1]).c_str());
+            ++g.ops;
+        }
+        for (u32 b = 0; b < 8; ++b) {
+            const u32 o = (r - r0) * 8 + b;
+            const std::vector<int> &pk = q.pk[b];
+            size_t i = 0;
+            if (!started[o] && !pk.empty()) {
+                if (pk.size() == 1) {
+                    g.line("            a%u = %s;", o, sig_name(pk[0]).c_str());
+                } else if (pk.size() == 2) {
+                    g.line("            a%u = %s ^ %s;", o, sig_name(pk[0]).c_str(),
+                           sig_name(pk[1]).c_str());
+                    ++g.ops;
+                } else {
+                    g.line("            a%u = xr3(%s, %s, %s);", o, sig_name(pk[0]).c_str(),
+                           sig_name(pk[1]).c_str(), sig_name(pk[2]).c_str());
+                    ++g.ops;
+                }
+                i = pk.size() < 3 ? pk.size() : 3;
+                started[o] = true;
+            }
+            for (; i < pk.size(); i += 2) {
+                if (i + 1 < pk.size())
+                    g.line("            a%u = xr3(a%u, %s, %s);", o, o, sig_name(pk[i]).c_str(),
+                           sig_name(pk[i + 1]).c_str());
+                else
+                    g.line("            a%u ^= %s;", o, sig_name(pk[i]).c_str());
+                ++g.ops;
+            }
+        }
+        g.line("        }");
+    }
+}
 
 void emit_program(Gen &g, int w, u32 k, u32 T, const uint8_t *coef, u32 r0, u32 r1)
 {
@@ -104,64 +246,14 @@
                 g.line("    n%d = LDW(col + %uu);", b, ((p + 1) * 8 + (u32)b) * ps);
         g.line("    __builtin_amdgcn_sched_barrier(0);");
         g.line("    {");
-        std::vector<u32> masks(no);
-        for (u32 o = 0; o < no; ++o)
-            masks[o] = plane_mask(coef[(size_t)(r0 + o / 8) * k + p], (int)(o % 8));
-        for (int h = 0; h < 2; ++h) {
-            bool need[16] = {};
-            for (u32 o = 0; o < no; ++o)
-                need[(masks[o] >> (4 * h)) & 15] = true;
-            bool have[16] = {};
-            for (int j = 0; j < 4; ++j) {
-                g.line("        const u32 t%d_%d = x%d;", h, 1 << j, 4 * h + j);
-                have[1 << j] = true;
-            }
-            for (int pc = 2; pc <= 4; ++pc)
-                for (int m = 1; m < 16; ++m) {
-                    if (__builtin_popcount(m) != pc || !(need[m] || (pc == 2 && m == 3 && need[15])))
-                        continue;
-                    if (have[m])
-                        continue;
-                    int bits[4], nb = 0;
-                    for (int j = 0; j < 4; ++j)
-                        if (m >> j & 1)
-                            bits[nb++] = 1 << j;
-                    if (pc == 2)
-                        g.line("        const u32 t%d_%d = t%d_%d ^ t%d_%d;", h, m, h, bits[0], h, bits[1]);
-                    else if (pc == 3)
-                        g.line("        const u32 t%d_%d = xr3(t%d_%d, t%d_%d, t%d_%d);", h, m, h, bits[0],
-                               h, bits[1], h, bits[2]);
-                    else
-                        g.line("        const u32 t%d_15 = xr3(t%d_3, t%d_4, t%d_8);", h, h, h, h);
-                    have[m] = true;
-                    ++g.ops;
-                }
-        }
-        for (u32 o = 0; o < no; ++o) {
-            const u32 m0 = masks[o] & 15, m1 = masks[o] >> 4;
-            char t0[16] = "", t1[16] = "";
-            if (m0)
-                snprintf(t0, sizeof t0, "t0_%u", m0);
-            if (m1)
-                snprintf(t1, sizeof t1, "t1_%u", m1);
-            if (!m0 && !m1)
-                continue;
-            if (!started[o]) {
-                if (m0 && m1) {
-                    g.line("        a%u = %s ^ %s;", o, t0, t1);
-                    ++g.ops;
-                } else {
-                    g.line("        a%u = %s;", o, m0 ? t0 : t1);
-                }
-                started[o] = true;
-            } else if (m0 && m1) {
-                g.line("        a%u = xr3(a%u, %s, %s);", o, o, t0, t1);
-                ++g.ops;
-            } else {
-                g.line("        a%u ^= %s;", o, m0 ? t0 : t1);
-                ++g.ops;
-            }
-        }
+        Gen tab, sea;
+        std::vector<bool> st_tab = started, st_sea = started;
+        emit_input_tables(tab, k, p, coef, r0, r1, st_tab);
+        emit_input_searched(sea, k, p, coef, r0, r1, st_sea);
+        const bool use_sea = sea.ops < tab.ops;
+        g.s += use_sea ? sea.s : tab.s;
+        g.ops += use_sea ? sea.ops : tab.ops;
+        started = use_sea ? st_sea : st_tab;
         g.line("    }");
         g.line("    __builtin_amdgcn_sched_barrier(0);");
     }
@@ -192,7 +284,8 @@
 __device__ __forceinline__ void body(const JitArgs &a)
 {
     extern __shared__ __attribute__((aligned(16))) unsigned char lds[];
-    constexpr u32 NW = T / 2u, PER = T / 2u, NT = NW * 64u;
+    /* a wave per 4 stripes and row group: G groups of R0 rows share a tile */
+    constexpr u32 NW = T / 4u * G, PER = T / 2u, NT = NW * 64u;
     const u32 tid = threadIdx.x, lane = tid & 63u;
     const u32 wave = __builtin_amdgcn_readfirstlane(tid >> 6);
     const u64 t0 = (u64)blockIdx.x * T;
@@ -213,20 +306,17 @@
      * build adds vmcnt(0) itself), so the wait is explicit */
     __builtin_amdgcn_s_waitcnt(0x0070);          /* vmcnt(0) lgkmcnt(0) */
     __syncthreads();
-    /* wave w: rows half (w & 1), stripes 4 * (w >> 1) .. + 3 */
-    const u32 half = wave & 1u, s = (wave >> 1) * 4u + (lane >> 4), cc = lane & 15u;
+    /* wave w: row group w % G, stripes 4 * (w / G) .. + 3 */
+    const u32 grp = wave % G, s = (wave / G) * 4u + (lane >> 4), cc = lane & 15u;
     const u32 col = (u32)(unsigned long long)(lds + s * 64u + cc * 4u);
     u32 acc[NA];
-    if (half == 0)
-        prog0(col, acc);
-    else
-        prog1(col, acc);
+    run_group(grp, col, acc);
     __syncthreads();
     /* stripe s, row r at (s * ROWS + r) * 512: a full decode's tile is then
      * its output as it lies in memory (ec_method_decode's stripe-major out) */
     unsigned char *ob = lds + s * (ROWS * 512u) + cc * 4u;
-    const u32 rb = half == 0 ? 0u : R0;
-    const u32 nr = half == 0 ? R0 : ROWS - R0;
+    const u32 rb = grp * R0;
+    const u32 nr = ROWS - rb < R0 ? ROWS - rb : R0;
 #pragma unroll
     for (u32 o = 0; o < NA; ++o)
         if (o < nr * 8u)
@@ -240,17 +330,18 @@
         for (u32 i = tid * 16u; i < ns * ROWS * 512u; i += NT * 16u)
             __builtin_nontemporal_store(*(const v4u *)(lds + i), (v4u *)(o + i));
     } else {
-        /* row by row: 512-byte runs, one per stripe (fragment-major outputs) */
-        for (u32 r = 0; r < ROWS; ++r) {
-            const u32 ss = tid >> 5, q = tid & 31u;
+        /* row by row: 512-byte runs, one per stripe (fragment-major outputs);
+         * with two row groups (NT = T * 32) one row per trip */
+        for (u32 i = tid; i < ROWS * T * 32u; i += NT) {
+            const u32 r = i / (T * 32u), ss = i / 32u % T, q = i & 31u;
             if (ss < ns)
                 __builtin_nontemporal_store(*(const v4u *)(lds + (ss * ROWS + r) * 512u + q * 16u),
                                             (v4u *)(a.out[r] + (t0 + ss) * a.out_stride + q * 16u));
         }
     }
 }
-extern "C" __global__ __launch_bounds__(T / 2 * 64) void ec_jit_combine(JitArgs a) { body<0>(a); }
-extern "C" __global__ __launch_bounds__(T / 2 * 64) void ec_jit_combine_nt(JitArgs a) { body<2>(a); }
+extern "C" __global__ __launch_bounds__(T / 4 * G * 64) void ec_jit_combine(JitArgs a) { body<0>(a); }
+extern "C" __global__ __launch_bounds__(T / 4 * G * 64) void ec_jit_combine_nt(JitArgs a) { body<2>(a); }
 )";
 
 
@@ -419,19 +510,67 @@
     return v;
 }
 
+constexpr long kNarrowMaxK = 8;
+constexpr long kNarrowMinStripes = 16384;
+
+u32 jit_narrow_max_k()
+{
+    static const long v = env_long("EC_MI355X_JIT_NARROW_MAX_K", kNarrowMaxK);
+    return v < 0 ? 0u : v > 8 ? 8u : (u32)v;
+}
+
+uint64_t jit_narrow_min_stripes()
+{
+    static const uint64_t v =
+        (uint64_t)env_long("EC_MI355X_JIT_NARROW_MIN_STRIPES", kNarrowMinStripes);
+    return v;
+}
+
+struct Shape {
+    u32 T, G, R0;
+};
+
+Shape shape_of(u32 k, u32 rows)
+{
+    Shape sh = {jit_tile(), 2, (rows + 1) / 2};
+    if (k > 8)
+        return sh;
+    static const long groups = env_long("EC_MI355X_JIT_NARROW_GROUPS", 4);
+    static const long tile = env_long("EC_MI355X_JIT_NARROW_TILE", 0);
+    sh.T = tile == 4 || tile == 8 || tile == 16 ? (u32)tile : k <= 4 ? 8u : 4u;
+    while (sh.T > 4 && (size_t)(k > rows ? k : rows) * sh.T * 512 > (64u << 10))
+        sh.T /= 2;
+    sh.G = groups == 1 || groups == 2 ? (u32)groups : 4u;
+    sh.R0 = (rows + sh.G - 1) / sh.G;
+    if ((sh.G - 1) * sh.R0 >= rows) {
+        sh.G = 2;
+        sh.R0 = (rows + 1) / 2;
+    }
+    return sh;
+}
+
 std::string source_of(const Key &key, u32 *ops)
 {
     Gen g;
-    const u32 r0 = (key.rows + 1) / 2;
+    const Shape sh = shape_of(key.k, key.rows);
     g.s += kPrologue;
     g.line("#define K %uu", key.k);
     g.line("#define ROWS %uu", key.rows);
-    g.line("#define R0 %uu", r0);
-    g.line("#define NA %uu", r0 * 8);
-    g.line("#define T %uu", jit_tile());
-
-    emit_program(g, 0, key.k, jit_tile(), key.coef, 0, r0);
-    emit_program(g, 1, key.k, jit_tile(), key.coef, r0, key.rows);
+    g.line("#define R0 %uu", sh.R0);
+    g.line("#define NA %uu", sh.R0 * 8);
+    g.line("#define T %uu", sh.T);
+    g.line("#define G %uu", sh.G);
+
+    for (u32 w = 0; w < sh.G; ++w) {
+        const u32 r0 = w * sh.R0, r1 = r0 + sh.R0 < key.rows ? r0 + sh.R0 : key.rows;
+        emit_program(g, (int)w, key.k, sh.T, key.coef, r0, r1);
+    }
+    g.line("__device__ __forceinline__ void run_group(u32 grp, u32 col, u32 *acc)");
+    g.line("{");
+    for (u32 w = 0; w + 1 < sh.G; ++w)
+        g.line("    %sif (grp == %uu)\n        prog%u(col, acc);", w ? "else " : "", w, w);
+    g.line("    %sprog%u(col, acc);", sh.G > 1 ? "else\n        " : "", sh.G - 1);
+    g.line("}");
     g.s += kBody;
     if (ops)
         *ops = g.ops;
@@ -581,10 +720,16 @@
 
 extern "C" int ecj_eligible(const ecd_combine_desc_t *d)
 {
-    if (!jit_on() || d->npatterns != 1 || d->group_pattern || d->k < 12 || d->k > ECJ_MAX ||
-        d->rows < 12 || d->rows > ECJ_MAX || d->nstripes < jit_min_stripes() ||
+    if (!jit_on() || d->npatterns != 1 || d->group_pattern || d->k > ECJ_MAX || d->rows > ECJ_MAX ||
         d->nstripes / 4 + 1 > 0x7fffffffull)
         return 0;
+    if (d->k <= 8) {
+        if (d->k < 1 || d->k > jit_narrow_max_k() || d->rows < 2 ||
+            d->nstripes < jit_narrow_min_stripes())
+            return 0;
+    } else if (d->k < 12 || d->rows < 12 || d->nstripes < jit_min_stripes()) {
+        return 0;
+    }
     if (d->out_stride % 16)
         return 0;
     for (uint32_t r = 0; r < d->rows; ++r)
@@ -624,14 +769,15 @@
     a.contig = d->out_stride == (uint64_t)d->rows * 512;
     for (uint32_t r = 1; r < d->rows && a.contig; ++r)
         a.contig = a.out[r] == a.out[0] + (size_t)r * 512;
-    const u32 T = jit_tile();
+    const Shape sh = shape_of(d->k, d->rows);
+    const u32 T = sh.T;
     const size_t lds = (size_t)(d->k > d->rows ? d->k : d->rows) * T * 512 +
                        (size_t)ecj_lds_pad_kb * 1024;
     if (lds > (64u << 10))
         return -EAGAIN;
     void *params[] = {&a};
-    const hipError_t rc = hipModuleLaunchKernel(f, (u32)((d->nstripes + T - 1) / T), 1, 1, T / 2 * 64,
-                                                1, 1, (u32)lds, s, params, nullptr);
+    const hipError_t rc = hipModuleLaunchKernel(f, (u32)((d->nstripes + T - 1) / T), 1, 1,
+                                                T / 4 * sh.G * 64, 1, 1, (u32)lds, s, params, nullptr);
     if (rc != hipSuccess) {
         (void)hipGetLastError();
         return -EAGAIN;
```
